# Zoe187419/ATE_replication_causalML

Measured on AMD Instinct MI355X. Metric: rows/sec for DML-ATE cross-fit, N=1e7 p=500, 1/2/4/8 MI355X; ATE/SE parity, higher is better.
Workload: dtype bf16; 1 GPU; model=DML-PLR 5-fold cross-fit, CV-LASSO nuisances (100 lambdas, inner 4-fold CV), global_batch=10000000, seq_len=500, N=10000000, p=500, folds=5, parallelism=dp1, dgp=tutorial, n_kept=10000000, layout=blocked64+bytes8

## Files before the change

ate_replication_causalml_amd/_native.py:

```python
from __future__ import annotations

import ctypes
import os
from pathlib import Path

_LIBDIR = Path(__file__).resolve().parent / "_lib"
_hip = None
_cpu = None


class NativeMissing(RuntimeError):
    pass


class NativeError(RuntimeError):

    def __init__(self, name: str, status: int, detail: str):
        self.entry, self.status = name, status
        super().__init__(f"{name} failed with status {status}: {detail}")


HIP_ERRORS = {
    1: "hipErrorInvalidValue", 2: "hipErrorOutOfMemory", 3: "hipErrorNotInitialized",
    4: "hipErrorDeinitialized", 9: "hipErrorInvalidConfiguration",
    13: "hipErrorInvalidSymbol", 17: "hipErrorInvalidDevicePointer",
    21: "hipErrorInvalidMemcpyDirection", 35: "hipErrorInsufficientDriver",
    52: "hipErrorMissingConfiguration", 53: "hipErrorPriorLaunchFailure",
    98: "hipErrorInvalidDeviceFunction", 100: "hipErrorNoDevice", 101: "hipErrorInvalidDevice",
    200: "hipErrorInvalidImage", 201: "hipErrorInvalidContext", 209: "hipErrorNoBinaryForGpu",
    218: "hipErrorInvalidKernelFile", 400: "hipErrorInvalidHandle", 500: "hipErrorNotFound",
    600: "hipErrorNotReady", 700: "hipErrorIllegalAddress", 701: "hipErrorLaunchOutOfResources",
    702: "hipErrorLaunchTimeOut", 710: "hipErrorAssert", 719: "hipErrorLaunchFailure",
    720: "hipErrorCooperativeLaunchTooLarge", 801: "hipErrorNotSupported",
    900: "hipErrorStreamCaptureUnsupported", 901: "hipErrorStreamCaptureInvalidated",
    907: "hipErrorCapturedEvent", 999: "hipErrorUnknown",
}


def describe_status(rc: int) -> str:
    if rc < 0:
        return "rejected by the entry point's own argument check (no kernel launched)"
    return f"{HIP_ERRORS.get(rc, 'hipError?')} ({rc})"


c_void_p = ctypes.c_void_p
c_int = ctypes.c_int
c_int64 = ctypes.c_int64
c_uint64 = ctypes.c_uint64
c_double = ctypes.c_double

_SIGS = {
    "ate_gram_bf16": "pliipipipipppp",
    "ate_gram_bf16_pair": "pllipippipippippiip",
    "ate_last_error": "pi",
    "ate_last_stale_error": "pi",
    "ate_clear_errors": "",
    "ate_debug_bad_launch": "ip",
    "ate_check_kernel_resources": "pi",
    "ate_gram_f32": "plippipipippppp",
    "ate_gram_f64": "plippipipippppp",
    "ate_gram_tile_sizes": "pppp",
    "ate_chol_solve": "pipiipdpppppp",
    "ate_chol_solve_k": "pipipidppppp",
    "ate_spd_solve_batched": "ppiippp",
    "ate_predict": "ipllppiidipp",
    "ate_irls_update": "ipllppiiiiippppipp",
    "ate_irls_check": "piidippp",
    "ate_naive": "ippplpppp",
    "ate_clip_propensity": "pplpp",
    "ate_aipw": "ppppppldpppp",
    "ate_dml_moments": "ppplppp",
    "ate_dml_finalize": "pipp",
    "ate_boot_multinomial": "ppluiipp",
    "ate_boot_poisson": "ppluiilipp",
    "ate_enet_prepare": "piipipiipipipppppppp",
    "ate_enet_prepare_fused": "piipipiipipi" + "ppppppp" + "plp",
    "ate_enet_prepare_fused_clear": "piipipiipipi" + "ppppppp" + "pl" + "pl" + "p",
    "ate_enet_path": "pipiippppidddipppppippp",
    "ate_enet_coef": "ppiiiipppppppp",
    "ate_enet_cvloss_gauss": "pippiipppiiipp",
    "ate_cv_select": "pppiipippppip",
    "ate_enet_pick": "ppiiipppip",
    "ate_enet_cv_tail": "pippiipppi" + "pppppp" + "iiii" + "pppppppppppp",
    "ate_dml_resid_moments": "ipllpipipiiiiiippp",
    "ate_dml_resid_moments_final": "ipllpipipiiiiii" + "ppppp",
    "ate_dml_resid_exact": "pllpipipiiiiiiippp",
    "ate_dml_resid_terms": "ipllpipipiiiiii" + "ppp",
    "ate_cluster_chunk": "",
    "ate_cluster_work": "l",
    "ate_cluster_moments": "pplpplipppp",
    "ate_irm_score_moments": "ipllpipiipiiiiidippp",
    "ate_irm_score_moments_multi": "ipllpipiipipiiiiiidippp",
    "ate_irm_score_multi_smax": "",
    "ate_irm_scores": "ipllpipiipiiiiidipp",
    "ate_irm_sens_moments": "ipllpipiipiiiiidippp",
    "ate_irm_target_moments": "ipllpipiipiiiiidippp",
    "ate_irm_score_link": "ii" + "ipllpipiipiiiiidippp",
    "ate_iivm_moments": "ipllpipiipiiiiiiidippp",
    "ate_apo_moments": "ipllpipiipiiiiidippp",
    "ate_pliv_lds_max": "",
    "ate_pliv_moments": "ipllpipiippii" + "pppp",
    "ate_pliv_terms": "ipllpipiippii" + "pppp",
    "ate_group_boot": "pppliiuippp",
    "ate_group_boot_scratch": "iii",
    "ate_cate_moments": "ppplpiiippp",
    "ate_cate_moments_scratch": "iii",
    "ate_cate_boot": "ppplppiiiuippp",
    "ate_cate_boot_scratch": "iiii",
    "ate_policy_pair_hist": "ppppppliiipp",
    "ate_policy_pair_hist_scratch": "i",
    "ate_policy_search": "ppiilppp",
    "ate_lognet_path": "iplpiipipipdddippippppppppp",
    "ate_lognet_cvloss": "iplpiippipppipp",
    "ate_lognet_path_groups": "iplpiipipipppdpdiippppppppp",
    "ate_lognet_cvloss_set": "iplpiipipipppipp",
    "ate_dgp_fill": "iplllllp" + "uiipppp",
    "ate_sel_block_rows": "",
    "ate_sel_gen_count": "upilllpp",
    "ate_sel_gen_flags": "upillpp",
    "ate_sel_gen_mark": "upiplllpiplp",
    "ate_forest_fit": "pppppi" + "pppppppp" + "ip",
    "ate_forest_predict": "ppiiipppppippip",
    "ate_forest_pack": "pippppppp",
    "ate_forest_scratch_bytes": "ii",
    "ate_forest_exact_scratch_bytes": "iiii",
    "ate_forest_fit_exact": "piiipppippppippppppppp",
    "ate_forest_predict16": "ppiiipppppppippip",
    "ate_bin_matrix": "plipppp",
    "ate_panel_xtv": "iplpipplipp",
    "ate_select_compact": "plppddpppp" + "p",
    "ate_gbdt_run": "ppp",
    "ate_lv_boot": "ppp",
    "ate_lv_classify": "pipiippp",
    "ate_lv_decide": "ppipipipippppp" + "iipip",
    "ate_lv_partition": "ppipippppipp",
    "ate_lv_scatter": "pppppippp",
    "ate_lv_children": "pippppp",
    "ate_lv_transpose": "piipip",
    "ate_gbdt_bin_panel": "pilpipppilpppl" + "p",
    "ate_gbdt_slab_entries": "liii",
    "ate_gbdt_slab2_entries": "li",
    "ate_gbdt_pair_root": "pppplllp",
    "ate_gbdt_apply": "plliipppp" + "p",
    "ate_panel_xv": "iplpipiplpp",
    "ate_col_moments": "pllipppp",
    "ate_standardize": "pllippp",
    "ate_interactions": "pllipl" + "p",
    "ate_scan_parts": "l",
    "ate_gbdt_limits": "p",
    "ate_excl_scan_i32": "plpppp",
    "ate_excl_scan_i64": "plpppp",
}
_RESTYPE = {"ate_forest_scratch_bytes": ctypes.c_int64,
            "ate_forest_exact_scratch_bytes": ctypes.c_int64, "ate_gbdt_slab_entries": ctypes.c_int64,
            "ate_gbdt_slab2_entries": ctypes.c_int64,
            "ate_scan_parts": ctypes.c_int64, "ate_group_boot_scratch": ctypes.c_int64,
            "ate_cate_moments_scratch": ctypes.c_int64,
            "ate_cate_boot_scratch": ctypes.c_int64,
            "ate_policy_pair_hist_scratch": ctypes.c_int64,
            "ate_cluster_work": ctypes.c_int64}
_CT = {"p": c_void_p, "i": c_int, "l": c_int64, "u": c_uint64, "d": c_double}


def _load(path: Path, sigs: dict):
    lib = ctypes.CDLL(str(path), mode=ctypes.RTLD_GLOBAL)
    for name, sig in sigs.items():
        if hasattr(lib, name):
            f = getattr(lib, name)
            f.restype = _RESTYPE.get(name, c_int)
            f.argtypes = [_CT[ch] for ch in sig]
    return lib


def hip_available() -> bool:
    return (_LIBDIR / "libatehip.so").exists()


def hip_library_path() -> Path:
    debug = os.environ.get("ATE_DEBUG", "0") not in ("", "0")
    return Path(os.environ["ATE_HIP_LIB"]) if os.environ.get("ATE_HIP_LIB") else \
        _LIBDIR / ("libatehip_debug.so" if debug else "libatehip.so")


def hip():
    global _hip
    if _hip is None:
        import torch
        debug = os.environ.get("ATE_DEBUG", "0") not in ("", "0")
        p = hip_library_path()
        if not p.exists():
            raise NativeMissing(
                f"{p} not found: build it with `python -m ate_replication_causalml_amd._build` "
                "(hipcc --offload-arch=gfx950). GPU ops have no fallback.")
        _hip = _load(p, _SIGS)
        if debug:
            _check_kernel_resources(_hip)
    return _hip


_resource_report = None


def _check_kernel_resources(lib):
    global _resource_report
    buf = ctypes.create_string_buffer(1 << 14)
    bad = lib.ate_check_kernel_resources(buf, len(buf))
    _resource_report = buf.value.decode(errors="replace")
    if bad > 0:
        raise NativeError("ate_check_kernel_resources", bad,
                          "kernels that cannot launch as registered:\n" + "\n".join(
                              l for l in _resource_report.splitlines() if "FAIL" in l))


def kernel_resource_report() -> str | None:
    return _resource_report


def _native_message(lib, fn: str) -> tuple[int, str]:
    buf = ctypes.create_string_buffer(512)
    code = getattr(lib, fn)(buf, len(buf))
    return code, buf.value.decode(errors="replace")


def cpu():
    global _cpu
    if _cpu is None:
        p = _LIBDIR / "libatecpu.so"
        if not p.exists():
            from ._build import build_cpu
            build_cpu()
        _cpu = _load(p, {})
    return _cpu


def check(rc: int, name: str = "native call"):
    if rc != 0:
        raise RuntimeError(f"{name} failed with code {rc}")


def call(name: str, *args):
    lib = hip()
    rc = getattr(lib, name)(*args)
    if rc != 0:
        raise NativeError(name, rc, status_detail(lib, rc))
    return rc


def status_detail(lib, rc: int) -> str:
    detail = describe_status(rc)
    if rc > 0 and hasattr(lib, "ate_last_error"):
        code, msg = _native_message(lib, "ate_last_error")
        if code == rc and msg:
            detail = msg
        scode, smsg = _native_message(lib, "ate_last_stale_error")
        if scode and smsg:
            detail += f" [stale, cleared before the launch: {smsg}]"
        lib.ate_clear_errors()
    return detail


def loaded_libraries():
    out = []
    try:
        with open(f"/proc/{os.getpid()}/maps") as f:
            for line in f:
                if str(_LIBDIR) in line:
                    out.append(line.split()[-1])
    except OSError:
        pass
    return sorted(set(out))
```

ate_replication_causalml_amd/data/device_dgp.py:

```python
from __future__ import annotations

import os

import numpy as np
import torch

from .. import _native
from ..ops.panel import DevicePanel, empty_panel, dtype_code
from . import dgp as host_dgp

N_TUTORIAL_COLS = 21
DGPS = ("tutorial", "tutorial-rct", "rct")


def fold_slices(n_total: int, folds: int, rank: int = 0, world: int = 1, align: int = 0):
    out = []
    for k in range(folds):
        f0, f1 = k * n_total // folds, (k + 1) * n_total // folds
        m = f1 - f0
        if align:
            nb = -(-m // align)
            a = min(f1, f0 + (rank * nb // world) * align)
            b = min(f1, f0 + ((rank + 1) * nb // world) * align)
        else:
            a = f0 + rank * m // world
            b = f0 + (rank + 1) * m // world
        out.append((a, b - a))
    return out


BYTE_COL0 = 384
BYTE_PANEL = os.environ.get("ATE_PANEL_BYTES", "1") == "1"


def _binary_names(p: int) -> set:
    out = {"one", "W", "Y", "W_hi", "W_lo", "Y_hi", "Y_lo"}
    out |= {f"x{j}" for j in range(15, min(21, p))}
    out |= {f"x{j}" for j in range(21, p) if (j - 21) % 4 == 3}
    return out


def byte_column_order(names: list, p: int, P: int):
    if P != 512:
        return None
    binary = _binary_names(p)
    cont = [nm for nm in names if nm not in binary]
    if len(cont) > BYTE_COL0:
        return None
    return cont + [nm for nm in names if nm in binary]


def _arm_split_ids(base: DevicePanel):
    w = base.col("W").double()
    counts, gparts, rows = [], [], []
    off = 0
    for (r0, _), cnt in zip(base.seg_bounds, base.seg_nreal):
        r0, cnt = int(r0), int(cnt)
        wk = w[r0:r0 + cnt]
        rk = base.row_index[r0:r0 + cnt]
        gk = rk if base.gen_ids is None else base.gen_ids[off:off + cnt]
        off += cnt
        for a in (0, 1):
            ix = torch.nonzero(wk == a).reshape(-1)
            counts.append(int(ix.numel()))
            gparts.append(gk[ix])
            rows.append(rk[ix])
    if sum(counts) != base.n:
        raise ValueError("arm_split needs a binary W column")
    return counts, torch.cat(gparts).contiguous(), rows, base.selection


def synthetic_panel(n_total: int, p: int = 500, folds: int = 5, seed: int = 1991,
                    dtype: str = "bf16", device="cpu", rank: int = 0, world: int = 1,
                    blocked: bool = False, align: int = 0, dgp: str = "rct", comm=None,
                    selection=None, compat: str = "reference",
                    arm_split: bool = False) -> DevicePanel:
    if p < N_TUTORIAL_COLS:
        raise ValueError("p must be >= 21 (tutorial columns)")
    if dgp not in DGPS:
        raise ValueError(f"dgp must be one of {DGPS}, got {dgp!r}")
    if comm is not None:
        rank, world = comm.rank, comm.world_size
    p_extra = p - N_TUTORIAL_COLS
    params = host_dgp.PANEL if dgp == "rct" else host_dgp.TUTORIAL
    if arm_split and align:
        raise ValueError("arm_split panels are not block-aligned: align must be 0")
    slices = fold_slices(n_total, folds, rank, world, align)
    split = None
    if arm_split:
        split = _arm_split_ids(synthetic_panel(
            n_total, p=p, folds=folds, seed=seed, dtype=dtype, device=device, rank=rank,
            world=world, blocked=blocked, dgp=dgp, comm=comm, selection=selection, compat=compat))
        slices = [(0, c) for c in split[0]]
    hi_lo = dtype == "bf16"
    names = ["one"] + [f"x{j}" for j in range(p)] + ["W", "Y"]
    if hi_lo:
        names += ["W_hi", "W_lo", "Y_hi", "Y_lo"]
    cpad = 128 if dtype == "bf16" else 64
    P = (len(names) + cpad - 1) // cpad * cpad
    pan = empty_panel([c for _, c in slices], P, dtype=dtype, device=device, blocked=blocked)
    order = byte_column_order(names, p, P) if (
        hi_lo and blocked and pan.data.is_cuda and BYTE_PANEL) else None
    pan.cols = {nm: i for i, nm in enumerate(names if order is None else order)}
    pan.xcols = [pan.cols[f"x{j}"] for j in range(p)]
    pcol = None
    if order is not None:
        pcol = torch.as_tensor([pan.cols[nm] for nm in names], dtype=torch.int16,
                               device=pan.data.device)
        pan.bytes8 = torch.zeros((pan.ld // 64, P - BYTE_COL0, 64), dtype=torch.uint8,
                                 device=pan.data.device)
    rid = torch.full((pan.ld,), -1, dtype=torch.int64, device=device)
    for (g0, cnt), (r0, _) in zip(slices, pan.seg_bounds):
        rid[r0:r0 + cnt] = torch.arange(g0, g0 + cnt, device=device)
    pan.row_index = rid
    pan.identity = len(slices) == 1 and slices[0][0] == 0
    gids = None
    sel = None
    if split is not None:
        _, gids, rows, sel = split
        for k, (r0, _) in enumerate(pan.seg_bounds):
            rid[r0:r0 + int(split[0][k])] = rows[k]
    elif dgp == "tutorial":
        from .panel_selection import kept_gids, plan_selection
        pcomm = None if getattr(comm, "emulated", False) else comm
        sel = selection if selection is not None else plan_selection(
            n_total, seed, params, comm=pcomm, device=pan.data.device, compat=compat)
        if sel.n_keep != n_total or sel.seed != seed:
            raise ValueError("selection plan does not match (n_total, seed)")
        if sel.compat != compat or sel.params != params:
            raise ValueError(f"selection plan made for compat={sel.compat!r} / other DGP "
                             f"parameters, not compat={compat!r}")
        gids = kept_gids(sel, slices, device=pan.data.device)
    offs = np.concatenate([[0], np.cumsum([c for _, c in slices])])
    if pan.data.is_cuda:
        s = torch.cuda.current_stream().cuda_stream
        pblk = np.ascontiguousarray(params.device_block())
        for k, ((g0, cnt), (r0, _)) in enumerate(zip(slices, pan.seg_bounds)):
            gp = 0 if gids is None or cnt == 0 else gids[int(offs[k]):].data_ptr()
            _native.call("ate_dgp_fill", dtype_code(pan.data), pan.data.data_ptr(),
                         *pan.strides(), int(r0), cnt, g0, gp, seed, p_extra, int(hi_lo),
                         pblk.ctypes.data, None if pcol is None else pcol.data_ptr(),
                         None if pcol is None else pan.bytes8.data_ptr(), s)
    else:
        cm = torch.zeros((pan.P, pan.ld), dtype=pan.data.dtype) if blocked else pan.data
        for k, ((g0, cnt), (r0, _)) in enumerate(zip(slices, pan.seg_bounds)):
            idx = None if gids is None else gids[int(offs[k]):int(offs[k]) + cnt].numpy()
            cts, binc, extra, W, Y, _ = host_dgp.raw_columns(cnt, seed, p_extra, row_offset=g0,
                                                              params=params, idx=idx)
            cols = [np.ones(cnt), *cts.T, *binc.T, *extra.T, W, Y]
            if hi_lo:
                cols += [W, np.zeros(cnt), Y, np.zeros(cnt)]
            block = torch.from_numpy(np.stack(cols)).to(pan.data.dtype)
            cm[:block.shape[0], r0:r0 + cnt] = block
        if blocked:
            pan.data.copy_(cm.reshape(pan.P, -1, 64).permute(1, 0, 2))
    pan.n = sum(c for _, c in slices)
    pan.exact_block = int(align)
    pan.dgp = dgp
    pan.selection = sel
    pan.n_generated = sel.n_gen if sel is not None else n_total
    pan.gen_ids = gids
    return pan
```

ate_replication_causalml_amd/ops/gram.py:

```python
from __future__ import annotations

import contextlib
import os

import numpy as np
import torch

from .. import _native
from ..utils.graphs import pin
from .panel import DevicePanel

BF16_TILE, BF16_K = 128, 64
BF16_TILE_BIG = 256
SMALL_TILE, SMALL_K = 64, 16
TARGET_WG = 2048

GRAM_KERNEL = os.environ.get("ATE_GRAM_KERNEL", "pair")
PAIR_SLOTS = 272
BYTE_COLS = os.environ.get("ATE_GRAM_BYTES", "1") == "1"
SCHEDULES = {"lockstep": 0, "stagger": 1}
GRAM_SCHED = os.environ.get("ATE_GRAM_SCHED", "stagger")
GRAM_PRIO = int(os.environ.get("ATE_GRAM_PRIO", "-1"))
PLAN_CACHE_MAX = int(os.environ.get("ATE_GRAM_PLAN_CACHE", 8))

_plan_cache: dict = {}
_slot = 0


@contextlib.contextmanager
def plan_slot(i: int):
    global _slot
    prev, _slot = _slot, int(i)
    try:
        yield
    finally:
        _slot = prev


def _stream():
    return torch.cuda.current_stream().cuda_stream


class GramPlan:
    def __init__(self, panel: DevicePanel, weighted: bool, exact: bool = False):
        bf16 = panel.dtype == torch.bfloat16
        if bf16 and weighted:
            raise ValueError("weighted Gram needs an fp32/fp64 panel")
        P = panel.P
        self.pair = bf16 and P % (2 * BF16_TILE_BIG) == 0 and GRAM_KERNEL == "pair"
        if bf16:
            T = BF16_TILE_BIG if P % BF16_TILE_BIG == 0 else BF16_TILE
        else:
            T = SMALL_TILE
        K = BF16_K if bf16 else SMALL_K
        if P % T:
            raise ValueError(f"panel P={P} must be a multiple of {T}")
        nt = P // T
        if self.pair:
            tiles, blocks = _pair_tiles(nt)
        else:
            tiles = [(a, b) for a in range(nt) for b in range(a, nt)]
        ntiles = len(tiles)
        rows_total = int((panel.seg_bounds[:, 1] - panel.seg_bounds[:, 0]).sum())
        target = 3072 if T == BF16_TILE_BIG else TARGET_WG
        whole_rounds = False
        if self.pair:
            env = os.environ.get("ATE_GRAM_PAIR_WG")
            whole_rounds = env is None
            rounds = int(os.environ.get("ATE_GRAM_ROUNDS", "5"))
            target = int(env) if env is not None else rounds * _cu_count(panel.device)
        target = int(os.environ.get("ATE_GRAM_WG", target))
        nchunk_target = max(1, target // ntiles)
        chunks = []
        seg_chunk0 = [0]
        if exact:
            B = int(panel.exact_block)
            if B <= 0 or B % K:
                raise ValueError("exact Gram needs a block-aligned panel (synthetic_panel("
                                 f"align=B) with B a multiple of {K})")
            for s_, (r0, r1) in enumerate(panel.seg_bounds):
                r = int(r0)
                while r < r1:
                    e = min(int(r1), r + B)
                    chunks.append((r, e, s_, 0))
                    r = e
                seg_chunk0.append(len(chunks))
        elif self.pair:
            chunks, seg_chunk0 = pair_chunks(panel.seg_bounds, K, ntiles, target,
                                             _cu_count(panel.device) if whole_rounds else 0)
        else:
            ch_rows = max(K, (rows_total // nchunk_target) // K * K)
            for s, (r0, r1) in enumerate(panel.seg_bounds):
                r = int(r0)
                while r < r1:
                    e = min(int(r1), r + ch_rows)
                    chunks.append((r, e, s, 0))
                    r = e
                seg_chunk0.append(len(chunks))
        dev = panel.device
        self.T, self.K, self.ntiles, self.nchunks = T, K, ntiles, len(chunks)
        self.tiles = torch.tensor(tiles, dtype=torch.int32, device=dev)
        if self.pair:
            self.blocks = torch.tensor(blocks, dtype=torch.int32, device=dev)
        ch = np.zeros(len(chunks), dtype=[("r0", "<i8"), ("r1", "<i8"), ("seg", "<i4"),
                                          ("pad", "<i4")])
        for i, c in enumerate(chunks):
            ch[i] = c
        self.chunks = torch.from_numpy(ch.view(np.uint8).copy()).to(dev)
        self.seg_chunk0 = torch.tensor(seg_chunk0, dtype=torch.int32, device=dev)
        slab_dtype = torch.float32 if panel.dtype != torch.float64 else torch.float64
        per_tile = PAIR_SLOTS * 256 if self.pair else T * T
        self.slab = torch.empty(self.nchunks * ntiles * per_tile, dtype=slab_dtype, device=dev)
        self.G = torch.empty((panel.nseg, P, P), dtype=torch.float64, device=dev)
        self.Gx = torch.empty((2, panel.nseg, P, P), dtype=torch.int64, device=dev) \
            if exact else None


def pair_chunks(seg_bounds, K: int, ntiles: int, target: int, ncu: int = 0):
    nseg = max(1, len(seg_bounds))
    k = max(1, max(1, target // ntiles) // nseg)
    if ncu > 0:
        per = ntiles * nseg
        kr = k
        while kr > 1 and (per * kr) % ncu:
            kr -= 1
        if (per * kr) % ncu == 0 and 2 * kr >= k:
            k = kr
    chunks, seg_chunk0 = [], [0]
    for s, (r0, r1) in enumerate(seg_bounds):
        r0, r1 = int(r0), int(r1)
        steps = (r1 - r0) // K
        ks = max(1, min(k, steps))
        for j in range(ks):
            a = r0 + (steps * j // ks) * K
            e = r0 + (steps * (j + 1) // ks) * K if j + 1 < ks else r1
            chunks.append((a, e, s, 0))
        seg_chunk0.append(len(chunks))
    return chunks, seg_chunk0


def _cu_count(dev) -> int:
    try:
        return int(torch.cuda.get_device_properties(dev).multi_processor_count)
    except Exception:
        return 256


def _pair_tiles(nt: int):
    tiles = []
    for a in range(0, nt - 1, 2):
        tiles.append((a, a + 1, 0, 0))
        tiles.append((a, a + 1, 1, 0))
    if nt % 2:
        tiles.append((nt - 1, nt - 1, 2, 0))
    paired = {(a, a + 1) for a in range(0, nt - 1, 2)}
    tiles += [(a, b, 0, 0) for a in range(nt) for b in range(a + 1, nt) if (a, b) not in paired]
    blocks = []
    for (a, b, typ, _) in tiles:
        tb = [(-1, -1)] * PAIR_SLOTS
        if typ == 0:
            for w in range(8):
                wr, wc = w >> 2, w & 3
                for m in range(8):
                    for n in range(4):
                        tb[w * 32 + m * 4 + n] = (a * 16 + wr * 8 + m, b * 16 + wc * 4 + n)
        else:
            rs, ts = 32, 36
            for w in range(4):
                region, half = w >> 1, w & 1
                if typ == 2 and region == 1:
                    continue
                base = (a if region == 0 else b) * 16
                for m in range(8):
                    for n in range(4):
                        tb[w * rs + m * 4 + n] = (base + m, base + 8 + half * 4 + n)
            for w in range(4):
                region, half = w >> 1, w & 1
                if typ == 2 and region == 1:
                    continue
                base = (a if region == 0 else b) * 16 + half * 8
                idx = 0
                for m in range(8):
                    for n in range(m, 8):
                        tb[4 * rs + w * ts + idx] = (base + m, base + n)
                        idx += 1
        blocks.append(tb)
    return tiles, blocks


def plan_for(panel: DevicePanel, weighted=False, exact=False) -> GramPlan:
    key = (panel.data.data_ptr(), tuple(panel.data.shape), panel.data.dtype, weighted,
           tuple(map(tuple, panel.seg_bounds)), _slot, exact)
    pl = _plan_cache.pop(key, None)
    if pl is None:
        while len(_plan_cache) >= PLAN_CACHE_MAX:
            _plan_cache.pop(next(iter(_plan_cache)))
        pl = GramPlan(panel, weighted, exact)
    _plan_cache[key] = pl
    return pin(pl)


def clear_plans():
    _plan_cache.clear()


_STAGES = {"all": 3, "tiles": 1, "reduce": 2}


def _sched_for(cs: int) -> int:
    return SCHEDULES[GRAM_SCHED] if cs < (1 << 28) else SCHEDULES["lockstep"]


EXACT_LIMB_BOUND = 2.0 ** 38


def check_exact_range(panel: DevicePanel, n_total: int | None = None, w=None, comm=None):
    X = panel.data
    if X.is_cuda and torch.cuda.is_current_stream_capturing():
        return
    dims = (0, 2) if panel.blocked else 1
    amax = torch.maximum(X.amax(dim=dims), -X.amin(dim=dims)).double()
    m = torch.stack([amax.max(), w.abs().max().double() if w is not None
                     else torch.ones((), dtype=torch.float64, device=amax.device)])
    if comm is not None and comm.world_size > 1:
        comm.all_reduce_max_(m)
    xm, wm = (float(v) for v in m.cpu())
    bound = xm ** 2 * float(n_total or panel.n)
    if w is not None:
        bound *= wm
    if not bound < EXACT_LIMB_BOUND:
        raise ValueError(f"exact Gram: entries up to {bound:.3g} exceed the int64 limb range "
                         f"(2^38 = {EXACT_LIMB_BOUND:.3g}); rescale the columns or use the "
                         "non-exact mode")


def gram(panel: DevicePanel, w: torch.Tensor | None = None, done: torch.Tensor | None = None,
         out: torch.Tensor | None = None, stage: str = "all", exact: bool = False,
         n_total: int | None = None, checked: bool = False) -> torch.Tensor:
    X = panel.data
    if exact and stage != "reduce" and not checked:
        check_exact_range(panel, n_total, w)
    if not X.is_cuda:
        if exact:
            return _gram_cpu_exact(panel, w)
        return _gram_cpu(panel, w, out) if stage != "reduce" else out
    pl = plan_for(panel, weighted=w is not None, exact=exact)
    G = pl.G if out is None else out
    Gx = pl.Gx.data_ptr() if exact else None
    s = _stream()
    if X.dtype == torch.bfloat16 and pl.pair:
        cs, bs = panel.strides()
        x8 = getattr(panel, "bytes8", None)
        _native.call("ate_gram_bf16_pair", X.data_ptr(), cs, bs, panel.P, pl.tiles.data_ptr(),
                     pl.ntiles, pl.blocks.data_ptr(), pl.chunks.data_ptr(), pl.nchunks,
                     pl.seg_chunk0.data_ptr(), panel.nseg, pl.slab.data_ptr(), G.data_ptr(),
                     _STAGES[stage], Gx, None if x8 is None or not BYTE_COLS else x8.data_ptr(),
                     _sched_for(cs), GRAM_PRIO, s)
        return pl.Gx if exact else G
    if stage == "reduce":
        return pl.Gx if exact else G
    if X.dtype == torch.bfloat16:
        _native.call("ate_gram_bf16", X.data_ptr(), panel.cm_ld, panel.P, pl.T, pl.tiles.data_ptr(),
                     pl.ntiles, pl.chunks.data_ptr(), pl.nchunks, pl.seg_chunk0.data_ptr(),
                     panel.nseg, pl.slab.data_ptr(), G.data_ptr(), Gx, s)
    else:
        name = "ate_gram_f64" if X.dtype == torch.float64 else "ate_gram_f32"
        if w is not None:
            assert w.dtype == X.dtype and w.numel() == panel.ld
        _native.call(name, X.data_ptr(), panel.cm_ld, panel.P, 0 if w is None else w.data_ptr(),
                     pl.tiles.data_ptr(), pl.ntiles, pl.chunks.data_ptr(), pl.nchunks,
                     pl.seg_chunk0.data_ptr(), panel.nseg, pl.slab.data_ptr(), G.data_ptr(),
                     0 if done is None else done.data_ptr(), Gx, s)
    return pl.Gx if exact else G


def _gram_cpu(panel, w, out):
    X = panel.colmajor().double()
    Gs = []
    for (r0, r1) in panel.seg_bounds:
        Xs = X[:, r0:r1]
        A = Xs if w is None else Xs * w[r0:r1].double()
        Gs.append(A @ Xs.T)
    G = torch.stack(Gs)
    if out is not None:
        out.copy_(G)
        return out
    return G


def _gram_cpu_exact(panel, w):
    from .exact import to_limbs
    B = int(panel.exact_block)
    if B <= 0:
        raise ValueError("exact Gram needs a block-aligned panel (synthetic_panel(align=B))")
    X = panel.colmajor().double()
    out = torch.zeros((2, panel.nseg, panel.P, panel.P), dtype=torch.int64)
    for s_, (r0, r1) in enumerate(panel.seg_bounds):
        for r in range(int(r0), int(r1), B):
            e = min(int(r1), r + B)
            Xs = X[:, r:e]
            A = Xs if w is None else Xs * w[r:e].double()
            out[:, s_] += to_limbs(A @ Xs.T)
    return out


def gram_reference(panel: DevicePanel, w=None) -> torch.Tensor:
    X = panel.colmajor().double().cpu()
    wv = None if w is None else w.double().cpu()
    out = []
    for (r0, r1) in panel.seg_bounds:
        Xs = X[:, r0:r1]
        A = Xs if wv is None else Xs * wv[r0:r1]
        out.append(A @ Xs.T)
    return torch.stack(out)
```

ate_replication_causalml_amd/ops/panel.py:

```python
from __future__ import annotations

from dataclasses import dataclass, field

import numpy as np
import torch

ROW_ALIGN = 64


def _dtype(name):
    return {"bf16": torch.bfloat16, "f32": torch.float32, "f64": torch.float64}[name]


def dtype_code(t: torch.Tensor) -> int:
    return {torch.float32: 1, torch.float64: 2, torch.bfloat16: 3}[t.dtype]


@dataclass
class DevicePanel:
    data: torch.Tensor
    n: int
    cols: dict
    seg_bounds: np.ndarray
    seg_nreal: np.ndarray
    row_index: torch.Tensor
    xcols: list = field(default_factory=list)
    identity: bool = False
    blocked: bool = False
    exact_block: int = 0
    bytes8: torch.Tensor | None = None

    @property
    def P(self):
        return self.data.shape[1] if self.blocked else self.data.shape[0]

    @property
    def ld(self):
        return self.data.shape[0] * ROW_ALIGN if self.blocked else self.data.shape[1]

    @property
    def cm_ld(self):
        if self.blocked:
            raise NotImplementedError("this kernel reads column-major panels only; build the "
                                      "panel with blocked=False")
        return self.data.shape[1]

    def strides(self):
        return (ROW_ALIGN, ROW_ALIGN * self.P) if self.blocked else (self.ld, ROW_ALIGN)

    @property
    def device(self):
        return self.data.device

    @property
    def dtype(self):
        return self.data.dtype

    @property
    def nseg(self):
        return len(self.seg_bounds)

    def col(self, name) -> torch.Tensor:
        c = self.cols[name]
        return self.data[:, c, :].reshape(-1) if self.blocked else self.data[c]

    def valid(self) -> torch.Tensor:
        return self.col("one")

    def colmajor(self) -> torch.Tensor:
        if not self.blocked:
            return self.data
        return self.data.permute(1, 0, 2).reshape(self.P, self.ld)

    def gather_rows(self, v: torch.Tensor) -> torch.Tensor:
        out = torch.zeros(self.ld, dtype=v.dtype, device=self.device)
        if self.identity:
            out[:self.n] = v.to(self.device)
            return out
        m = self.row_index >= 0
        out[m] = v.to(self.device)[self.row_index[m]]
        return out

    def scatter_rows(self, v: torch.Tensor) -> torch.Tensor:
        if self.identity:
            return v[:self.n].clone()
        m = self.row_index >= 0
        out = torch.empty((self.n,) + tuple(v.shape[1:]), dtype=v.dtype, device=v.device)
        out[self.row_index[m]] = v[m]
        return out


def _round_up(x, m):
    return (x + m - 1) // m * m


def build_panel(X, W=None, Y=None, folds=None, dtype="f64", device="cpu", extra_cols=(),
                col_align=None, split_hi_lo=None, nseg=None, targets=None) -> DevicePanel:
    Xt = None
    if isinstance(X, torch.Tensor):
        Xt = X.to(device=device, dtype=torch.float64)
        if Xt.ndim == 1:
            Xt = Xt[:, None]
        X = np.empty(tuple(Xt.shape), dtype=np.float64)
    X = np.asarray(X, dtype=np.float64)
    if X.ndim == 1:
        X = X[:, None]
    n, p = X.shape
    tdt = _dtype(dtype)
    if split_hi_lo is None:
        split_hi_lo = dtype == "bf16"
    if col_align is None:
        col_align = 128 if dtype == "bf16" else 64
    names = ["one"] + [f"x{j}" for j in range(p)]
    vecs = {}
    if W is not None:
        names.append("W")
        vecs["W"] = np.asarray(W, float)
    if Y is not None:
        names.append("Y")
        vecs["Y"] = np.asarray(Y, float)
    if split_hi_lo:
        for k in list(vecs):
            names += [f"{k}_hi", f"{k}_lo"]
    for k, v in (targets or {}).items():
        if k in names or k in extra_cols or len(np.shape(v)) != 1 or len(v) != n:
            raise ValueError(f"target column {k!r}: a new name and {n} values are needed")
        names.append(k)
        vecs[k] = np.asarray(v, float)
        if split_hi_lo:
            names += [f"{k}_hi", f"{k}_lo"]
    names += list(extra_cols)
    P = _round_up(len(names), col_align)
    if folds is None:
        folds = np.zeros(n, dtype=np.int64)
    folds = np.asarray(folds, dtype=np.int64)
    K = max(int(folds.max()) + 1 if n else 1, int(nseg or 0))
    order = np.argsort(folds, kind="stable")
    counts = np.bincount(folds, minlength=K)
    padded = np.array([_round_up(max(c, 1), ROW_ALIGN) for c in counts])
    starts = np.concatenate([[0], np.cumsum(padded)[:-1]])
    ld = int(padded.sum())
    row_index = np.full(ld, -1, dtype=np.int64)
    pos = 0
    for k in range(K):
        rows = order[pos:pos + counts[k]]
        row_index[starts[k]:starts[k] + counts[k]] = rows
        pos += counts[k]
    m = row_index >= 0
    ri = row_index[m]
    host = np.zeros((P if Xt is None else P - p, ld), dtype=np.float64)
    hrow = (lambda r: r) if Xt is None else (lambda r: r if r == 0 else r - p)
    host[0, m] = 1.0
    if Xt is None:
        host[1:1 + p, m] = X[ri].T
    c = 1 + p
    cols = {n_: i for i, n_ in enumerate(names)}
    for k, v in vecs.items():
        host[hrow(cols[k]), m] = v[ri]
    if split_hi_lo:
        for k, v in vecs.items():
            hi = torch.from_numpy(v[ri]).to(torch.bfloat16).double().numpy()
            lo = v[ri] - hi
            host[hrow(cols[f"{k}_hi"]), m] = hi
            host[hrow(cols[f"{k}_lo"]), m] = lo
    if Xt is None:
        data = torch.from_numpy(host).to(tdt).to(device)
    else:
        data = torch.empty((P, ld), dtype=tdt, device=device)
        rest = torch.from_numpy(host).to(tdt).to(device)
        data[:1] = rest[:1]
        data[1 + p:] = rest[1:]
        blk = torch.zeros((p, ld), dtype=torch.float64, device=device)
        blk[:, torch.from_numpy(np.flatnonzero(m)).to(device)] = \
            Xt[torch.from_numpy(ri).to(device)].T
        data[1:1 + p] = blk.to(tdt)
    seg_bounds = np.stack([starts, starts + padded], axis=1)
    return DevicePanel(data=data, n=n, cols=cols, seg_bounds=seg_bounds,
                       seg_nreal=counts.astype(np.int64),
                       row_index=torch.from_numpy(row_index).to(device),
                       xcols=[cols[f"x{j}"] for j in range(p)], identity=K == 1)


def empty_panel(n_per_seg, P, dtype="bf16", device="cpu", blocked=False):
    counts = np.asarray(n_per_seg, dtype=np.int64)
    padded = np.array([_round_up(max(int(c), 1), ROW_ALIGN) for c in counts])
    starts = np.concatenate([[0], np.cumsum(padded)[:-1]])
    ld = int(padded.sum())
    shape = (ld // ROW_ALIGN, P, ROW_ALIGN) if blocked else (P, ld)
    data = torch.zeros(shape, dtype=_dtype(dtype), device=device)
    row_index = torch.full((ld,), -1, dtype=torch.int64, device=device)
    base = 0
    for s, c in zip(starts, counts):
        row_index[s:s + c] = torch.arange(base, base + c, device=device)
        base += int(c)
    return DevicePanel(data=data, n=int(counts.sum()), cols={"one": 0},
                       seg_bounds=np.stack([starts, starts + padded], axis=1),
                       seg_nreal=counts, row_index=row_index, identity=len(counts) == 1,
                       blocked=blocked)
```

ate_replication_causalml_amd/utils/graphs.py:

```python
from __future__ import annotations

import contextlib
import gc

import torch

_pins: list | None = None


@contextlib.contextmanager
def _no_gc():
    was = gc.isenabled()
    gc.disable()
    try:
        yield
    finally:
        if was:
            gc.enable()


def pin(obj):
    if _pins is not None:
        _pins.append(obj)
    return obj


class GraphedStep:
    def __init__(self, fn, warmup: int = 1):
        global _pins
        self.fn = fn
        for _ in range(warmup):
            fn()
        torch.cuda.synchronize()
        self.graph = torch.cuda.CUDAGraph()
        prev, _pins = _pins, []
        try:
            gc.collect()
            with _no_gc(), torch.cuda.graph(self.graph):
                self.out = fn()
            self.pins = _pins
        finally:
            _pins = prev
        torch.cuda.synchronize()

    def __call__(self):
        self.graph.replay()
        return self.out


def maybe_graphed(fn, enable: bool, warmup: int = 1):
    if not enable or not torch.cuda.is_available():
        return fn, False
    try:
        return GraphedStep(fn, warmup), True
    except Exception as e:
        print(f"[graphs] capture failed, running eagerly: {e}", flush=True)
        torch.cuda.synchronize()
        return fn, False


class Collective:

    def __init__(self, fn, capturable: bool = False):
        self.fn = fn
        self.capturable = capturable

    def __call__(self, state):
        return self.fn(state)


def _fuse(phases, fuse_collectives=False):
    out, run = [], []

    def flush():
        if run:
            fns = tuple(run)

            def composed(st, fns=fns):
                for f in fns:
                    st = f(st)
                return st
            out.append(composed)
            run.clear()

    for ph in phases:
        if isinstance(ph, Collective) and not (fuse_collectives and ph.capturable):
            flush()
            out.append(ph)
        else:
            run.append(ph)
    flush()
    return out


class SegmentedStep:

    def __init__(self, phases, graph: bool, warmup: int = 1, capture_collectives: bool = True,
                 agree=None):
        self.raw = list(phases)
        self.fallback_reason = None
        has_cc = any(isinstance(p, Collective) and p.capturable for p in self.raw)
        self.phases = _fuse(self.raw)
        self.graphs = [None] * len(self.phases)
        self.pins = []
        self.collectives_captured = False
        for _ in range(warmup):
            self._eager()
        if not graph:
            return
        if capture_collectives and has_cc:
            ok, err = True, None
            try:
                self._capture(_fuse(self.raw, fuse_collectives=True), replay=False)
            except Exception as e:
                ok, err = False, e
            if agree is not None:
                ok = bool(agree(ok))
                if err is None and not ok:
                    err = RuntimeError("another rank could not capture its collectives")
            if ok:
                self()
                torch.cuda.synchronize()
                self.collectives_captured = True
                return
            self.fallback_reason = repr(err)
            print(f"[graphs] capturing the collectives failed, they run eagerly between "
                  f"graph segments: {err}", flush=True)
            torch.cuda.synchronize()
            self.phases = _fuse(self.raw)
            self.graphs = [None] * len(self.phases)
            self.pins = []
        self._capture(_fuse(self.raw))

    def _capture(self, phases, replay: bool = True):
        global _pins
        torch.cuda.synchronize()
        graphs = [None] * len(phases)
        pins = []
        state = None
        for i, ph in enumerate(phases):
            if isinstance(ph, Collective):
                state = ph(state)
                continue
            g = torch.cuda.CUDAGraph()
            prev, _pins = _pins, []
            try:
                gc.collect()
                with _no_gc(), torch.cuda.graph(g):
                    out = ph(state)
                pins += _pins
            finally:
                _pins = prev
            graphs[i] = (g, out)
            torch.cuda.synchronize()
            if replay:
                g.replay()
            state = out
        torch.cuda.synchronize()
        self.phases, self.graphs, self.pins = phases, graphs, pins

    @property
    def graphed(self) -> bool:
        return any(g is not None for g in self.graphs)

    @property
    def graph_count(self) -> int:
        return sum(g is not None for g in self.graphs)

    def _eager(self):
        state = None
        for ph in self.phases:
            state = ph(state)
        return state

    def __call__(self):
        state = None
        for ph, g in zip(self.phases, self.graphs):
            if g is None:
                state = ph(state)
            else:
                g[0].replay()
                state = g[1]
        return state


def _data(x):
    return x if isinstance(x, torch.Tensor) else x.data


def layout_key(*inputs):
    key = []
    for x in inputs:
        if x is None:
            key.append(None)
            continue
        t = _data(x)
        k = (tuple(t.shape), t.dtype, str(t.device))
        if not isinstance(x, torch.Tensor):
            k += (x.n, tuple(sorted(x.cols.items())), tuple(map(tuple, x.seg_bounds)),
                  tuple(int(c) for c in x.seg_nreal), bool(getattr(x, "identity", False)),
                  getattr(x, "bytes8", None) is not None)
        key.append(k)
    return tuple(key)


class _Captured:

    def __init__(self, body, inputs, static_args, warmup):
        self.inputs = inputs = list(inputs)
        self.step = GraphedStep(lambda: body(*inputs, *static_args), warmup)

    def load(self, inputs):
        for s, x in zip(self.inputs, inputs):
            if x is not s and x is not None:
                _data(s).copy_(_data(x))
                if getattr(x, "bytes8", None) is not None:
                    s.bytes8.copy_(x.bytes8)

    def __call__(self, inputs):
        self.load(inputs)
        return self.step()


class _Seen:

    def __init__(self, inputs):
        self.inputs = None if inputs is None else list(inputs)


def _nbytes(inputs):
    tot = 0
    for x in inputs:
        if x is None:
            continue
        t = _data(x)
        tot += t.numel() * t.element_size()
    return tot


def _env_bytes(name, default):
    import os
    v = os.environ.get(name)
    return int(float(v)) if v else default


class GraphCache:

    def __init__(self, maxsize: int = 32, max_bytes: int | None = None,
                 retain_bytes: int | None = None):
        self.maxsize = maxsize
        self.max_bytes = max_bytes if max_bytes is not None else \
            _env_bytes("ATE_GRAPH_CACHE_BYTES", 24 << 30)
        self.retain_bytes = retain_bytes if retain_bytes is not None else \
            _env_bytes("ATE_GRAPH_RETAIN_BYTES", 1 << 30)
        self.entries: dict = {}
        self.sizes: dict = {}
        self.eager: set = set()

    @property
    def held_bytes(self):
        return sum(self.sizes.values())

    def _evict(self, need=0):
        while self.entries and (len(self.entries) >= self.maxsize or
                                self.held_bytes + need > self.max_bytes):
            k = next(iter(self.entries))
            self.entries.pop(k)
            self.sizes.pop(k, None)

    def run(self, name, body, inputs, *static_args):
        key = (name, static_args, layout_key(*inputs))
        if key in self.eager:
            return body(*inputs, *static_args), False
        g = self.entries.pop(key, None)
        self.sizes.pop(key, None)
        nb = _nbytes(inputs)
        if g is None:
            keep = nb <= self.retain_bytes and nb <= self.max_bytes
            self._evict(nb if keep else 0)
            self.entries[key] = _Seen(inputs if keep else None)
            self.sizes[key] = nb if keep else 0
            return body(*inputs, *static_args), False
        if isinstance(g, _Seen):
            if nb > self.max_bytes:
                self.entries[key] = g
                self.sizes[key] = 0
                return body(*inputs, *static_args), False
            self._evict(nb)
            static = g.inputs if g.inputs is not None else list(inputs)
            try:
                torch.cuda.synchronize()
                for s, x in zip(static, inputs):
                    if x is not s and x is not None:
                        _data(s).copy_(_data(x))
                        if getattr(x, "bytes8", None) is not None:
                            s.bytes8.copy_(x.bytes8)
                g = _Captured(body, static, static_args, warmup=1)
            except Exception as e:
                print(f"[graphs] {name}: capture failed, running eagerly: {e}", flush=True)
                torch.cuda.synchronize()
                self.eager.add(key)
                return body(*inputs, *static_args), False
        self.entries[key] = g
        self.sizes[key] = nb
        return g(inputs), True

    def drop(self, name, inputs, *static_args):
        key = (name, static_args, layout_key(*inputs))
        self.entries.pop(key, None)
        self.sizes.pop(key, None)
        self.eager.discard(key)

    def clear(self):
        self.entries.clear()
        self.sizes.clear()
        self.eager.clear()


estimator_graphs = GraphCache()


def clear_graph_caches():
    estimator_graphs.clear()
    try:
        from ..ops.gram import clear_plans
        clear_plans()
    except Exception:
        pass
    if torch.cuda.is_available():
        torch.cuda.empty_cache()
```

csrc/dgp.hip:

```cpp
#include "common.hpp"

using namespace ate;

namespace {

struct DgpP {
  float intercept, b_hist[5], b_latent, tau_logit, p_treat, thr[5], hist_latent, yob_latent,
      factor_load, factor_rest;
  int uniform_b;
  double p_treat_d, thr_d[5], hist_latent_d, yob_latent_d;
};

DgpP load_params(const double* a) {
  DgpP P;
  P.p_treat_d = a[8];
  for (int k = 0; k < 5; ++k) P.thr_d[k] = a[9 + k];
  P.hist_latent_d = a[14];
  P.yob_latent_d = a[15];
  P.intercept = a[0];
  for (int k = 0; k < 5; ++k) P.b_hist[k] = a[1 + k];
  P.b_latent = a[6];
  P.tau_logit = a[7];
  P.p_treat = a[8];
  for (int k = 0; k < 5; ++k) P.thr[k] = a[9 + k];
  P.hist_latent = a[14];
  P.yob_latent = a[15];
  P.factor_load = a[16];
  P.factor_rest = a[17];
  P.uniform_b = 1;
  for (int k = 1; k < 5; ++k) P.uniform_b &= (P.b_hist[k] == P.b_hist[0]);
  return P;
}

__device__ __forceinline__ float dgp_normal(uint64_t seed, uint32_t stream, uint64_t idx) {
  u32x4 w = rand4(seed, P_DGP, stream, idx);
  float u1 = ((float)(w.x >> 8) + 1.0f) * (1.0f / 16777217.0f);
  float u2 = (float)(w.y >> 8) * (1.0f / 16777216.0f);
  return sqrtf(-2.0f * logf(u1)) * cosf(6.283185307179586f * u2);
}
__device__ __forceinline__ float dgp_uniform(uint64_t seed, uint32_t stream, uint64_t idx) {
  u32x4 w = rand4(seed, P_DGP, stream, idx);
  return (float)(w.x >> 8) * (1.0f / 16777216.0f);
}
__device__ __forceinline__ double dgp_normal_d(uint64_t seed, uint32_t stream, uint64_t idx) {
#pragma clang fp contract(off)
  u32x4 w = rand4(seed, P_DGP, stream, idx);
  const double u1 = ((double)(w.x >> 8) + 1.0) * (1.0 / 16777217.0);
  const double u2 = (double)(w.y >> 8) * (1.0 / 16777216.0);
  return sqrt(-2.0 * log(u1)) * cos(6.283185307179586 * u2);
}
__device__ __forceinline__ double dgp_uniform_d(uint64_t seed, uint32_t stream, uint64_t idx) {
  u32x4 w = rand4(seed, P_DGP, stream, idx);
  return (double)(w.x >> 8) * (1.0 / 16777216.0);
}

struct Core {
  double yob, city, latent;
  float w;
  int hist;
};

__device__ __forceinline__ Core core_draws(uint64_t seed, uint64_t g, const DgpP& P) {
#pragma clang fp contract(off)
  Core c;
  c.yob = dgp_normal_d(seed, 0, g);
  c.city = dgp_normal_d(seed, 1, g);
  c.latent = dgp_normal_d(seed, 41, g) + P.yob_latent_d * c.yob;
  c.hist = 0;
#pragma unroll
  for (int k = 0; k < 5; ++k)
    c.hist |= (dgp_normal_d(seed, 50 + k, g) + P.hist_latent_d * c.latent > P.thr_d[k])
                  ? (1 << k) : 0;
  c.w = dgp_uniform_d(seed, 61, g) < P.p_treat_d ? 1.f : 0.f;
  return c;
}

__device__ __forceinline__ int sel_flag(const Core& c, int last) {
  const int h = c.hist;
  if (c.w == 1.f) {
    const bool d = (h & 0xF) != 0 || ((h >> last) & 1) || c.city > 2.0 || c.yob > 2.0;
    return d ? 1 : 0;
  }
  const bool d = (h & 0x1F) != 0x1F || c.city < -2.0 || c.yob < -2.0;
  return d ? 2 : 0;
}

__device__ __forceinline__ int64_t pidx(int c, int64_t i, int64_t cs, int64_t bs) {
  return (int64_t)c * cs + (i >> 6) * bs + (i & 63);
}
template <typename T>
__device__ __forceinline__ void put(T* X, int64_t cs, int64_t bs, int c, int64_t i, float v) {
  X[pidx(c, i, cs, bs)] = (T)v;
}
template <>
__device__ __forceinline__ void put<bf16_t>(bf16_t* X, int64_t cs, int64_t bs, int c, int64_t i,
                                            float v) {
  X[pidx(c, i, cs, bs)] = f32_to_bf16_rne(v);
}
template <typename T>
__device__ __forceinline__ void put_d(T* X, int64_t cs, int64_t bs, int c, int64_t i, double v) {
  if constexpr (sizeof(T) == 8) X[pidx(c, i, cs, bs)] = (T)v;
  else put(X, cs, bs, c, i, (float)v);
}

constexpr int X8_COL0 = 384;
__device__ __forceinline__ int x8_pos(int64_t i) {
  const int r = (int)(i & 63);
  return ((r >> 3) & 3) * 16 + (r >> 5) * 8 + (r & 7);
}

template <typename T>
__global__ void dgp_fill_kernel(T* __restrict__ X, int64_t cs, int64_t bs, int64_t row0, int64_t count,
                                int64_t gid0, const int64_t* __restrict__ gids, uint64_t seed,
                                int p_extra, int hi_lo, DgpP P, const int16_t* __restrict__ pcol,
                                uint8_t* __restrict__ X8) {
  const float FL = P.factor_load, FS = P.factor_rest;
  for (int64_t r = blockIdx.x * (int64_t)blockDim.x + threadIdx.x; r < count;
       r += (int64_t)gridDim.x * blockDim.x) {
    const uint64_t g = gids != nullptr ? (uint64_t)gids[r] : (uint64_t)(gid0 + r);
    const int64_t i = row0 + r;
    const Core cr = core_draws(seed, g, P);
    const float f = dgp_normal(seed, 40, g);
    int c = 0;
    auto phys = [&](int cl) { return pcol != nullptr ? (int)pcol[cl] : cl; };
    auto emit = [&](float v) {
      const int pc = phys(c++);
      put(X, cs, bs, pc, i, v);
      if (X8 != nullptr && pc >= X8_COL0) {
        ATE_DASSERT(v == 0.f || v == 1.f);
        X8[(i >> 6) * (128 * 64) + (pc - X8_COL0) * 64 + x8_pos(i)] = v != 0.f ? 0x3F : 0;
      }
    };
    emit(1.0f);
    ATE_DASSERT(phys(1) < X8_COL0 || X8 == nullptr);
    put_d(X, cs, bs, phys(c++), i, cr.yob);
    put_d(X, cs, bs, phys(c++), i, cr.city);
    for (int j = 2; j < 15; ++j) {
      float z = dgp_normal(seed, j, g);
      emit(j < 3 ? z : FL * f + FS * z);
    }
    const float sex = dgp_uniform(seed, 60, g) < 0.5f ? 1.f : 0.f;
    emit(sex);
    float hsum = 0.f, hb = 0.f;
#pragma unroll
    for (int k = 0; k < 5; ++k) {
      const float h = ((cr.hist >> k) & 1) ? 1.f : 0.f;
      hsum += h;
      hb += P.b_hist[k] * h;
      emit(h);
    }
    for (int j = 0; j < p_extra; ++j) {
      float z = dgp_normal(seed, 100 + j, g);
      float v = (j % 4 == 3) ? (z > 0.f ? 1.f : 0.f) : FL * f + FS * z;
      emit(v);
    }
    const float w = cr.w;
    const float hterm = P.uniform_b ? P.b_hist[0] * hsum : hb;
    const float eta = P.intercept + hterm + P.b_latent * (float)cr.latent + P.tau_logit * w;
    const float y = dgp_uniform(seed, 62, g) < 1.0f / (1.0f + expf(-eta)) ? 1.f : 0.f;
    emit(w);
    emit(y);
    if (hi_lo) {
      emit(w);
      emit(0.f);
      emit(y);
      emit(0.f);
    }
  }
}

constexpr int NT = 256;
constexpr int SEL_BR = 16384;

__global__ __launch_bounds__(NT) void sel_gen_count_kernel(uint64_t seed, DgpP P, int last,
                                                           int64_t b0, int64_t n_lim,
                                                           int64_t* __restrict__ cnt) {
  __shared__ int ws[2][NT / 64];
  const int64_t b = b0 + blockIdx.x;
  const int64_t g0 = b * SEL_BR;
  int ct = 0, cc = 0;
  for (int k = threadIdx.x; k < SEL_BR; k += NT) {
    const int64_t g = g0 + k;
    if (g >= n_lim) break;
    const int f = sel_flag(core_draws(seed, (uint64_t)g, P), last);
    ct += f == 1;
    cc += f == 2;
  }
  ct = wave_sum(ct);
  cc = wave_sum(cc);
  const int lane = threadIdx.x & 63, wid = threadIdx.x >> 6;
  if (lane == 0) { ws[0][wid] = ct; ws[1][wid] = cc; }
  __syncthreads();
  if (threadIdx.x == 0) {
    int64_t t = 0, c = 0;
    for (int w = 0; w < NT / 64; ++w) { t += ws[0][w]; c += ws[1][w]; }
    cnt[2 * blockIdx.x] = t;
    cnt[2 * blockIdx.x + 1] = c;
  }
}

__global__ __launch_bounds__(NT) void sel_gen_flags_kernel(uint64_t seed, DgpP P, int last,
                                                           int64_t g0, int64_t count,
                                                           uint8_t* __restrict__ flags) {
  for (int64_t r = blockIdx.x * (int64_t)NT + threadIdx.x; r < count; r += (int64_t)gridDim.x * NT)
    flags[r] = (uint8_t)sel_flag(core_draws(seed, (uint64_t)(g0 + r), P), last);
}

__device__ int block_scan(int x, int* ws) {
  const int lane = threadIdx.x & 63, wid = threadIdx.x >> 6;
  int incl = x;
#pragma unroll
  for (int o = 1; o < 64; o <<= 1) {
    const int t = __shfl_up(incl, o, 64);
    if (lane >= o) incl += t;
  }
  if (lane == 63) ws[wid] = incl;
  __syncthreads();
  int off = 0, tot = 0;
  for (int w = 0; w < NT / 64; ++w) {
    if (w < wid) off += ws[w];
    tot += ws[w];
  }
  __syncthreads();
  if (threadIdx.x == 0) ws[NT / 64] = tot;
  __syncthreads();
  return off + incl - x;
}

__global__ __launch_bounds__(NT) void sel_gen_mark_kernel(uint64_t seed, DgpP P, int last,
                                                          const int64_t* __restrict__ blk,
                                                          int64_t thr_t, int64_t thr_c,
                                                          const int64_t* __restrict__ sl, int ns,
                                                          int64_t* __restrict__ out, int64_t cap) {
  __shared__ int ws[3][NT / 64 + 1];
  const int64_t* B = blk + 6 * (int64_t)blockIdx.x;
  const int64_t g0 = B[0], g1 = B[1];
  int64_t ct = B[2], cc = B[3], kp = B[4];
  ATE_DASSERT(g1 - g0 <= SEL_BR && g0 <= g1);
  for (int64_t base = g0; base < g1; base += NT) {
    const int64_t g = base + threadIdx.x;
    const int f = g < g1 ? sel_flag(core_draws(seed, (uint64_t)g, P), last) : 0;
    const int et = block_scan(f == 1, ws[0]);
    const int ec = block_scan(f == 2, ws[1]);
    const bool drop = (f == 1 && ct + et < thr_t) || (f == 2 && cc + ec < thr_c);
    const int k = g < g1 && !drop;
    const int ek = block_scan(k, ws[2]);
    if (k) {
      const int64_t q = kp + ek;
      for (int s = 0; s < ns; ++s) {
        if (q >= sl[3 * s] && q < sl[3 * s + 1]) {
          const int64_t o = sl[3 * s + 2] + (q - sl[3 * s]);
          ATE_DASSERT(o >= 0 && o < cap);
          out[o] = g;
          break;
        }
      }
    }
    ct += ws[0][NT / 64];
    cc += ws[1][NT / 64];
    kp += ws[2][NT / 64];
  }
}

}

ATE_API int ate_dgp_fill(int dtype, void* X, int64_t cs, int64_t bs, int64_t row0, int64_t count,
                         int64_t gid0, const void* gids, uint64_t seed, int p_extra, int hi_lo,
                         const void* params, const void* pcol, void* X8, void* stream) {
  hipStream_t s = (hipStream_t)stream;
  const DgpP P = load_params((const double*)params);
  const int64_t* gl = (const int64_t*)gids;
  const int16_t* pc = (const int16_t*)pcol;
  dim3 grid(grid_for(count, 256, 8192)), block(256);
  if (X8 != nullptr && dtype != 3) return -1;
  if (dtype == 1)
    ATE_LAUNCH(dgp_fill_kernel<float>, grid, block, 0, s, (float*)X, cs, bs, row0, count, gid0,
                       gl, seed, p_extra, hi_lo, P, pc, (uint8_t*)nullptr);
  else if (dtype == 2)
    ATE_LAUNCH(dgp_fill_kernel<double>, grid, block, 0, s, (double*)X, cs, bs, row0, count,
                       gid0, gl, seed, p_extra, hi_lo, P, pc, (uint8_t*)nullptr);
  else if (dtype == 3)
    ATE_LAUNCH(dgp_fill_kernel<bf16_t>, grid, block, 0, s, (bf16_t*)X, cs, bs, row0, count,
                       gid0, gl, seed, p_extra, hi_lo, P, pc, (uint8_t*)X8);
  else
    return -1;
  ATE_CHECK_LAUNCH();
  return 0;
}

ATE_API int ate_sel_block_rows() { return SEL_BR; }

ATE_API int ate_sel_gen_count(uint64_t seed, const void* params, int last, int64_t b0, int64_t nblk,
                              int64_t n_lim, void* cnt, void* stream) {
  if (nblk <= 0) return 0;
  const DgpP P = load_params((const double*)params);
  ATE_LAUNCH(sel_gen_count_kernel, dim3((unsigned)nblk), dim3(NT), 0, (hipStream_t)stream,
                     seed, P, last, b0, n_lim, (int64_t*)cnt);
  ATE_CHECK_LAUNCH();
  return 0;
}

ATE_API int ate_sel_gen_flags(uint64_t seed, const void* params, int last, int64_t g0, int64_t count,
                              void* flags, void* stream) {
  if (count <= 0) return 0;
  const DgpP P = load_params((const double*)params);
  ATE_LAUNCH(sel_gen_flags_kernel, dim3(grid_for(count, NT, 4096)), dim3(NT), 0,
                     (hipStream_t)stream, seed, P, last, g0, count, (uint8_t*)flags);
  ATE_CHECK_LAUNCH();
  return 0;
}

ATE_API int ate_sel_gen_mark(uint64_t seed, const void* params, int last, const void* blk, int64_t nl,
                             int64_t thr_t, int64_t thr_c, const void* sl, int ns, void* out,
                             int64_t cap, void* stream) {
  if (nl <= 0) return 0;
  const DgpP P = load_params((const double*)params);
  ATE_LAUNCH(sel_gen_mark_kernel, dim3((unsigned)nl), dim3(NT), 0, (hipStream_t)stream,
                     seed, P, last, (const int64_t*)blk, thr_t, thr_c, (const int64_t*)sl, ns,
                     (int64_t*)out, cap);
  ATE_CHECK_LAUNCH();
  return 0;
}
```

csrc/gram.hip:

```cpp
#include "common.hpp"

using namespace ate;

struct Chunk { int64_t row0, row1; int seg, pad; };

__device__ __forceinline__ int xcd_remap(int bid, int nwg) {
  int xcd = bid & 7, q = nwg >> 3, r = nwg & 7;
  int base = (xcd < r) ? xcd * (q + 1) : r * (q + 1) + (xcd - r) * q;
  return base + (bid >> 3);
}

constexpr int BT = 128;
constexpr int BK = 64;

__global__ __launch_bounds__(256) void gram_bf16_kernel(
    const bf16_t* __restrict__ X, int64_t ld, const int2* __restrict__ tiles, int ntiles,
    const Chunk* __restrict__ chunks, int nchunks, float* __restrict__ slab) {
  __shared__ __attribute__((aligned(16))) bf16_t lds[2][2][BT * BK];
  const int L = xcd_remap(blockIdx.x, gridDim.x);
  const int c = L / ntiles, t = L % ntiles;
  const Chunk ch = chunks[c];
  const int2 tl = tiles[t];
  const bool diag = tl.x == tl.y;
  const int a0 = tl.x * BT, b0 = tl.y * BT;
  const int tid = threadIdx.x, lane = tid & 63, wid = tid >> 6;
  const int wr = wid >> 1, wc = wid & 1;

  f32x4 acc[4][4];
#pragma unroll
  for (int i = 0; i < 4; ++i)
#pragma unroll
    for (int j = 0; j < 4; ++j) acc[i][j] = f32x4{0.f, 0.f, 0.f, 0.f};

  uint4 ra[4], rb[4];
  auto gload = [&](int64_t i0) {
#pragma unroll
    for (int r = 0; r < 4; ++r) {
      int idx = r * 256 + tid, col = idx >> 3, cc = idx & 7;
      ra[r] = *reinterpret_cast<const uint4*>(X + (int64_t)(a0 + col) * ld + i0 + cc * 8);
      if (!diag) rb[r] = *reinterpret_cast<const uint4*>(X + (int64_t)(b0 + col) * ld + i0 + cc * 8);
    }
  };
  auto lstore = [&](int buf) {
#pragma unroll
    for (int r = 0; r < 4; ++r) {
      int idx = r * 256 + tid, col = idx >> 3, cc = idx & 7;
      int off = col * BK + ((cc ^ (col & 7)) << 3);
      *reinterpret_cast<uint4*>(&lds[buf][0][off]) = ra[r];
      if (!diag) *reinterpret_cast<uint4*>(&lds[buf][1][off]) = rb[r];
    }
  };

  const int64_t nsteps = (ch.row1 - ch.row0) / BK;
  if (nsteps > 0) {
    gload(ch.row0);
    lstore(0);
  }
  __syncthreads();
  for (int64_t s = 0; s < nsteps; ++s) {
    const int buf = s & 1;
    if (s + 1 < nsteps) gload(ch.row0 + (s + 1) * BK);
    const bf16_t* As = lds[buf][0];
    const bf16_t* Bs = diag ? lds[buf][0] : lds[buf][1];
#pragma unroll
    for (int kk = 0; kk < 2; ++kk) {
      const int cc = kk * 4 + (lane >> 4);
      bf16x8 af[4], bfr[4];
#pragma unroll
      for (int m = 0; m < 4; ++m) {
        int col = wr * 64 + m * 16 + (lane & 15);
        af[m] = *reinterpret_cast<const bf16x8*>(&As[col * BK + ((cc ^ (col & 7)) << 3)]);
      }
#pragma unroll
      for (int n = 0; n < 4; ++n) {
        int col = wc * 64 + n * 16 + (lane & 15);
        bfr[n] = *reinterpret_cast<const bf16x8*>(&Bs[col * BK + ((cc ^ (col & 7)) << 3)]);
      }
#pragma unroll
      for (int m = 0; m < 4; ++m)
#pragma unroll
        for (int n = 0; n < 4; ++n)
          acc[m][n] = __builtin_amdgcn_mfma_f32_16x16x32_bf16(af[m], bfr[n], acc[m][n], 0, 0, 0);
    }
    if (s + 1 < nsteps) lstore(buf ^ 1);
    __syncthreads();
  }
  float* out = slab + ((int64_t)c * ntiles + t) * (BT * BT);
#pragma unroll
  for (int m = 0; m < 4; ++m)
#pragma unroll
    for (int n = 0; n < 4; ++n)
#pragma unroll
      for (int r = 0; r < 4; ++r) {
        int row = wr * 64 + m * 16 + (lane >> 4) * 4 + r;
        int col = wc * 64 + n * 16 + (lane & 15);
        out[row * BT + col] = acc[m][n][r];
      }
}

constexpr int GT = 256;
constexpr int GK = 64;

typedef const __attribute__((address_space(1))) char* gptr_t;
__device__ __forceinline__ void glds16(gptr_t src, bf16_t* lds_base) {
  __builtin_amdgcn_global_load_lds(src, (__attribute__((address_space(3))) void*)(lds_base), 16, 0, 0);
}
__device__ __forceinline__ void glds16(const void* src, bf16_t* lds_base) {
  __builtin_amdgcn_global_load_lds(src, (__attribute__((address_space(3))) void*)(lds_base), 16, 0, 0);
}

__global__ __launch_bounds__(512) void gram_bf16_256_kernel(
    const bf16_t* __restrict__ X, int64_t ld, const int2* __restrict__ tiles, int ntiles,
    const Chunk* __restrict__ chunks, int nchunks, float* __restrict__ slab) {
  __shared__ __attribute__((aligned(16))) bf16_t lds[2][2][GT * GK];
  const int L = xcd_remap(blockIdx.x, gridDim.x);
  const int c = L / ntiles, t = L % ntiles;
  const Chunk ch = chunks[c];
  const int2 tl = tiles[t];
  const bool diag = tl.x == tl.y;
  const int a0 = tl.x * GT, b0 = tl.y * GT;
  const int tid = threadIdx.x, lane = tid & 63, wid = tid >> 6;
  const int wr = wid >> 2, wc = wid & 3;

  f32x4 acc[8][4];
#pragma unroll
  for (int i = 0; i < 8; ++i)
#pragma unroll
    for (int j = 0; j < 4; ++j) acc[i][j] = f32x4{0.f, 0.f, 0.f, 0.f};

  auto stage = [&](int st, int64_t i0) {
#pragma unroll
    for (int r = 0; r < 4; ++r) {
      const int q = wid * 4 + r;
      const int col = q * 8 + (lane >> 3);
      const int cc = (lane & 7) ^ (col & 7);
      glds16(X + (int64_t)(a0 + col) * ld + i0 + cc * 8, &lds[st][0][q * 8 * GK]);
      if (!diag) glds16(X + (int64_t)(b0 + col) * ld + i0 + cc * 8, &lds[st][1][q * 8 * GK]);
    }
  };

  const int64_t nsteps = (ch.row1 - ch.row0) / GK;
  if (nsteps > 0) stage(0, ch.row0);
  __builtin_amdgcn_s_waitcnt(0x0F70);
  __syncthreads();
  for (int64_t s = 0; s < nsteps; ++s) {
    const int cur = s & 1;
    if (s + 1 < nsteps) stage(cur ^ 1, ch.row0 + (s + 1) * GK);
    const bf16_t* As = lds[cur][0];
    const bf16_t* Bs = diag ? lds[cur][0] : lds[cur][1];
#pragma unroll
    for (int kk = 0; kk < 2; ++kk) {
      const int cc = kk * 4 + (lane >> 4);
      bf16x8 af[8], bfr[4];
#pragma unroll
      for (int m = 0; m < 8; ++m) {
        const int col = wr * 128 + m * 16 + (lane & 15);
        af[m] = *reinterpret_cast<const bf16x8*>(&As[col * GK + ((cc ^ (col & 7)) << 3)]);
      }
#pragma unroll
      for (int n = 0; n < 4; ++n) {
        const int col = wc * 64 + n * 16 + (lane & 15);
        bfr[n] = *reinterpret_cast<const bf16x8*>(&Bs[col * GK + ((cc ^ (col & 7)) << 3)]);
      }
#pragma unroll
      for (int m = 0; m < 8; ++m)
#pragma unroll
        for (int n = 0; n < 4; ++n)
          acc[m][n] = __builtin_amdgcn_mfma_f32_16x16x32_bf16(af[m], bfr[n], acc[m][n], 0, 0, 0);
    }
    __builtin_amdgcn_s_waitcnt(0x0F70);
    __syncthreads();
  }
  float* out = slab + ((int64_t)c * ntiles + t) * (GT * GT);
#pragma unroll
  for (int m = 0; m < 8; ++m)
#pragma unroll
    for (int n = 0; n < 4; ++n)
#pragma unroll
      for (int r = 0; r < 4; ++r) {
        const int row = wr * 128 + m * 16 + (lane >> 4) * 4 + r;
        const int col = wc * 64 + n * 16 + (lane & 15);
        out[row * GT + col] = acc[m][n][r];
      }
}

constexpr int PAIR_SLOTS = 272;
constexpr int PAIR_LDS = 2 * 2 * GT * GK;
#ifndef GRAM_PRIO
#define GRAM_PRIO 2
#endif

__device__ __forceinline__ int tri_index(int m, int n) {
  return m * 8 - (m * (m - 1)) / 2 + (n - m);
}

constexpr int PAIR_RECT = 0, PAIR_RECT_D0 = 1, PAIR_TRI = 2, PAIR_RECT_D1 = 3;
template <int MODE> struct PairRole {
  static constexpr bool TRI = MODE == PAIR_TRI;
  static constexpr int NB = TRI ? 36 : 32;
};

template <int MODE>
__device__ __forceinline__ void pair_mfma(f32x4* acc, const bf16x8* af, const bf16x8* bfr) {
  if constexpr (MODE != PAIR_TRI) {
#pragma unroll
    for (int m = 0; m < 8; ++m)
#pragma unroll
      for (int n = 0; n < 4; ++n)
        acc[m * 4 + n] = __builtin_amdgcn_mfma_f32_16x16x32_bf16(af[m], bfr[n], acc[m * 4 + n],
                                                                 0, 0, 0);
  } else {
#pragma unroll
    for (int m = 0; m < 8; ++m)
#pragma unroll
      for (int n = m; n < 8; ++n)
        acc[tri_index(m, n)] = __builtin_amdgcn_mfma_f32_16x16x32_bf16(
            af[m], af[n], acc[tri_index(m, n)], 0, 0, 0);
  }
}

__device__ __forceinline__ bf16x8 bytes_to_bf16x8(uint2 d) {
  uint4 w;
  w.x = __builtin_amdgcn_perm(0u, d.x, 0x010C000Cu);
  w.y = __builtin_amdgcn_perm(0u, d.x, 0x030C020Cu);
  w.z = __builtin_amdgcn_perm(0u, d.y, 0x010C000Cu);
  w.w = __builtin_amdgcn_perm(0u, d.y, 0x030C020Cu);
  return __builtin_bit_cast(bf16x8, w);
}
constexpr int PAIR_BYTE0 = 384;

constexpr int SCHED_LOCKSTEP = 0, SCHED_STAGGER = 1;

template <int MODE, bool BYTES, bool BY, bool LATE, bool SADDR>
__device__ __forceinline__ void pair_wave(const bf16_t* __restrict__ X, int64_t cs, int64_t bs, int a0,
                                          int b0, bool haveB, bool idle, int abuf, int bbuf,
                                          int arow0, int bcol0, const Chunk& ch,
                                          bf16_t* lds_raw, float* __restrict__ out,
                                          const uint8_t* __restrict__ X8) {
  constexpr bool TRI = PairRole<MODE>::TRI;
  constexpr int NB = PairRole<MODE>::NB;
  const int tid = threadIdx.x, lane = tid & 63, wid = tid >> 6;
  f32x4 acc[NB];
#pragma unroll
  for (int i = 0; i < NB; ++i) acc[i] = f32x4{0.f, 0.f, 0.f, 0.f};
  bf16_t (*lds)[2][GT * GK] = reinterpret_cast<bf16_t (*)[2][GT * GK]>(lds_raw);
  const int wu = __builtin_amdgcn_readfirstlane(wid);
  const uint32_t voff_ = (uint32_t)(((lane >> 3) * cs + (((lane & 7) ^ (lane >> 3)) << 3)) * 2);
  const uint32_t voff8_ = (uint32_t)((lane >> 2) * GK + (((lane & 3) ^ ((lane >> 3) & 2)) << 4));
  auto stage = [&](int st, int64_t i0) {
    if constexpr (SADDR) {
      gptr_t Xk0 = (gptr_t) reinterpret_cast<const char*>(X + (i0 >> 6) * bs);
      uint32_t voff = voff_, voff8 = voff8_;
#if defined(__HIP_DEVICE_COMPILE__)
      asm volatile("" : "+v"(voff), "+v"(voff8));
#endif
      const int nbp = 2;
#pragma unroll
      for (int r = 0; r < 4; ++r) {
        const int q = wu * 4 + r;
        glds16(Xk0 + (int64_t)(a0 + q * 8) * cs * 2 + voff, &lds[st][0][q * 8 * GK]);
        if (!BYTES && haveB)
          glds16(Xk0 + (int64_t)(b0 + q * 8) * cs * 2 + voff, &lds[st][1][q * 8 * GK]);
      }
      if constexpr (BYTES) {
#pragma unroll
        for (int r = 0; r < nbp; ++r) {
          const int q = wu * 2 + r;
          glds16(Xk0 + (int64_t)(b0 + q * 8) * cs * 2 + voff, &lds[st][1][q * 8 * GK]);
        }
        glds16((gptr_t) reinterpret_cast<const char*>(X8) + (i0 >> 6) * (128 * GK) + wu * 1024 + voff8,
               reinterpret_cast<bf16_t*>(reinterpret_cast<uint8_t*>(&lds[st][1][128 * GK]) +
                                         wu * 1024));
      }
      return;
    }
    if constexpr (BYTES) {
      const bf16_t* Xk0 = X + (i0 >> 6) * bs;
#pragma unroll
      for (int r = 0; r < 4; ++r) {
        const int q = wid * 4 + r;
        const int col = q * 8 + (lane >> 3);
        const int cc = (lane & 7) ^ (col & 7);
        glds16(Xk0 + cc * 8 + (int64_t)(a0 + col) * cs, &lds[st][0][q * 8 * GK]);
      }
#pragma unroll
      for (int r = 0; r < 2; ++r) {
        const int q = wid * 2 + r;
        const int col = q * 8 + (lane >> 3);
        const int cc = (lane & 7) ^ (col & 7);
        glds16(Xk0 + cc * 8 + (int64_t)(b0 + col) * cs, &lds[st][1][q * 8 * GK]);
      }
      const int cb = wid * 16 + (lane >> 2);
      const int pc = (lane & 3) ^ ((cb >> 1) & 2);
      glds16(X8 + (i0 >> 6) * (128 * GK) + cb * GK + pc * 16,
             reinterpret_cast<bf16_t*>(reinterpret_cast<uint8_t*>(&lds[st][1][128 * GK]) +
                                       wid * 1024));
      return;
    }
#pragma unroll
    for (int r = 0; r < 4; ++r) {
      const int q = wid * 4 + r;
      const int col = q * 8 + (lane >> 3);
      const int cc = (lane & 7) ^ (col & 7);
      const bf16_t* Xk = X + (i0 >> 6) * bs + cc * 8;
      glds16(Xk + (int64_t)(a0 + col) * cs, &lds[st][0][q * 8 * GK]);
      if (haveB) glds16(Xk + (int64_t)(b0 + col) * cs, &lds[st][1][q * 8 * GK]);
    }
  };
  auto frag = [&](const bf16_t* P_, int col, int cc) {
    return *reinterpret_cast<const bf16x8*>(&P_[col * GK + ((cc ^ (col & 7)) << 3)]);
  };
  auto raw16 = [&](const bf16_t* P_, int col) {
    const int cb = col - 128;
    const uint8_t* b8 = reinterpret_cast<const uint8_t*>(P_ + 128 * GK);
    const int slot = (lane >> 4) ^ ((cb >> 1) & 2);
    return *reinterpret_cast<const uint4*>(b8 + cb * GK + slot * 16);
  };
  const int64_t nsteps = (ch.row1 - ch.row0) / GK;
  if (nsteps > 0) stage(0, ch.row0);
  __builtin_amdgcn_s_waitcnt(0x0F70);
  __syncthreads();
  bf16x8 ha[LATE ? 8 : 1], hb[LATE && !TRI ? 4 : 1];
  if constexpr (LATE) {
#pragma unroll
    for (int m = 0; m < 8; ++m) ha[m] = bf16x8{};
    if constexpr (!TRI) {
#pragma unroll
      for (int n = 0; n < 4; ++n) hb[n] = bf16x8{};
    }
  }
  for (int64_t s = 0; s < nsteps; ++s) {
    const int cur = s & 1;
    const bf16_t* As = lds[cur][abuf];
    const bf16_t* Bs = lds[cur][bbuf];
    if constexpr (LATE) {
      bf16x8 na[8], nb[TRI ? 1 : 4];
      uint4 raw[BY ? (TRI ? 8 : 4) : 1];
      const int c0 = lane >> 4, c1 = 4 + (lane >> 4);
      if (!idle) {
        if constexpr (BY && !TRI) {
#pragma unroll
          for (int n = 0; n < 4; ++n) raw[n] = raw16(Bs, bcol0 + n * 16 + (lane & 15));
#pragma unroll
          for (int m = 0; m < 8; ++m) na[m] = frag(As, arow0 + m * 16 + (lane & 15), c0);
          pair_mfma<MODE>(acc, ha, hb);
#pragma unroll
          for (int i = 0; i < 12; ++i) {
            __builtin_amdgcn_sched_group_barrier(0x008, 1, 0);
            __builtin_amdgcn_sched_group_barrier(0x100, 1, 0);
          }
          __builtin_amdgcn_sched_group_barrier(0x008, NB - 12, 0);
        } else if constexpr (BY) {
#pragma unroll
          for (int m = 0; m < 8; ++m) raw[m] = raw16(As, arow0 + m * 16 + (lane & 15));
#pragma unroll
          for (int m = 0; m < 8; ++m) na[m] = bytes_to_bf16x8(make_uint2(raw[m].x, raw[m].y));
          pair_mfma<MODE>(acc, ha, ha);
#pragma unroll
          for (int i = 0; i < 8; ++i) {
            __builtin_amdgcn_sched_group_barrier(0x008, 1, 0);
            __builtin_amdgcn_sched_group_barrier(0x100, 1, 0);
          }
#pragma unroll
          for (int i = 0; i < 16; ++i) {
            __builtin_amdgcn_sched_group_barrier(0x008, 1, 0);
            __builtin_amdgcn_sched_group_barrier(0x002, 2, 0);
          }
          __builtin_amdgcn_sched_group_barrier(0x008, NB - 24, 0);
        } else if constexpr (!TRI) {
#pragma unroll
          for (int m = 0; m < 8; ++m) na[m] = frag(As, arow0 + m * 16 + (lane & 15), c0);
#pragma unroll
          for (int n = 0; n < 4; ++n) nb[n] = frag(Bs, bcol0 + n * 16 + (lane & 15), c0);
          pair_mfma<MODE>(acc, ha, hb);
#pragma unroll
          for (int i = 0; i < 12; ++i) {
            __builtin_amdgcn_sched_group_barrier(0x008, 1, 0);
            __builtin_amdgcn_sched_group_barrier(0x100, 1, 0);
          }
          __builtin_amdgcn_sched_group_barrier(0x008, NB - 12, 0);
        } else {
#pragma unroll
          for (int m = 0; m < 8; ++m) na[m] = frag(As, arow0 + m * 16 + (lane & 15), c0);
          pair_mfma<MODE>(acc, ha, ha);
#pragma unroll
          for (int i = 0; i < 8; ++i) {
            __builtin_amdgcn_sched_group_barrier(0x008, 1, 0);
            __builtin_amdgcn_sched_group_barrier(0x100, 1, 0);
          }
          __builtin_amdgcn_sched_group_barrier(0x008, NB - 8, 0);
        }
      }
      if (s + 1 < nsteps) stage(cur ^ 1, ch.row0 + (s + 1) * GK);
      if (!idle) {
        if constexpr (BY && !TRI) {
#pragma unroll
          for (int m = 0; m < 8; ++m) ha[m] = frag(As, arow0 + m * 16 + (lane & 15), c1);
#pragma unroll
          for (int n = 0; n < 4; ++n) nb[n] = bytes_to_bf16x8(make_uint2(raw[n].x, raw[n].y));
#pragma unroll
          for (int n = 0; n < 4; ++n) hb[n] = bytes_to_bf16x8(make_uint2(raw[n].z, raw[n].w));
          pair_mfma<MODE>(acc, na, nb);
          __builtin_amdgcn_sched_group_barrier(0x002, 4, 0);
#pragma unroll
          for (int i = 0; i < 3; ++i) {
            __builtin_amdgcn_sched_group_barrier(0x008, 1, 0);
            __builtin_amdgcn_sched_group_barrier(0x002, 4, 0);
          }
#pragma unroll
          for (int i = 0; i < 8; ++i) {
            __builtin_amdgcn_sched_group_barrier(0x008, 1, 0);
            __builtin_amdgcn_sched_group_barrier(0x100, 1, 0);
          }
#pragma unroll
          for (int i = 0; i < 16; ++i) {
            __builtin_amdgcn_sched_group_barrier(0x008, 1, 0);
            __builtin_amdgcn_sched_group_barrier(0x002, 1, 0);
          }
          __builtin_amdgcn_sched_group_barrier(0x008, NB - 27, 0);
        } else if constexpr (BY) {
#pragma unroll
          for (int m = 0; m < 8; ++m) ha[m] = bytes_to_bf16x8(make_uint2(raw[m].z, raw[m].w));
          pair_mfma<MODE>(acc, na, na);
#pragma unroll
          for (int i = 0; i < 16; ++i) {
            __builtin_amdgcn_sched_group_barrier(0x008, 1, 0);
            __builtin_amdgcn_sched_group_barrier(0x002, 2, 0);
          }
          __builtin_amdgcn_sched_group_barrier(0x008, NB - 16, 0);
        } else if constexpr (!TRI) {
#pragma unroll
          for (int m = 0; m < 8; ++m) ha[m] = frag(As, arow0 + m * 16 + (lane & 15), c1);
#pragma unroll
          for (int n = 0; n < 4; ++n) hb[n] = frag(Bs, bcol0 + n * 16 + (lane & 15), c1);
          pair_mfma<MODE>(acc, na, nb);
#pragma unroll
          for (int i = 0; i < 12; ++i) {
            __builtin_amdgcn_sched_group_barrier(0x008, 1, 0);
            __builtin_amdgcn_sched_group_barrier(0x100, 1, 0);
          }
          __builtin_amdgcn_sched_group_barrier(0x008, NB - 12, 0);
        } else {
#pragma unroll
          for (int m = 0; m < 8; ++m) ha[m] = frag(As, arow0 + m * 16 + (lane & 15), c1);
          pair_mfma<MODE>(acc, na, na);
#pragma unroll
          for (int i = 0; i < 8; ++i) {
            __builtin_amdgcn_sched_group_barrier(0x008, 1, 0);
            __builtin_amdgcn_sched_group_barrier(0x100, 1, 0);
          }
          __builtin_amdgcn_sched_group_barrier(0x008, NB - 8, 0);
        }
      }
    } else {
      if (s + 1 < nsteps) stage(cur ^ 1, ch.row0 + (s + 1) * GK);
      if (!idle) {
        if constexpr (BY && !TRI) {
          bf16x8 af[2][8];
          uint4 braw[4];
#pragma unroll
          for (int n = 0; n < 4; ++n) braw[n] = raw16(Bs, bcol0 + n * 16 + (lane & 15));
#pragma unroll
          for (int kk = 0; kk < 2; ++kk) {
            const int cc = kk * 4 + (lane >> 4);
#pragma unroll
            for (int m = 0; m < 8; ++m) af[kk][m] = frag(As, arow0 + m * 16 + (lane & 15), cc);
          }
          bf16x8 b0v[4], b1v[4];
#pragma unroll
          for (int n = 0; n < 4; ++n) b0v[n] = bytes_to_bf16x8(make_uint2(braw[n].x, braw[n].y));
#pragma unroll
          for (int n = 0; n < 4; ++n) b1v[n] = bytes_to_bf16x8(make_uint2(braw[n].z, braw[n].w));
          pair_mfma<MODE>(acc, af[0], b0v);
          pair_mfma<MODE>(acc, af[1], b1v);
          __builtin_amdgcn_sched_group_barrier(0x100, 12, 0);
          __builtin_amdgcn_sched_group_barrier(0x002, 16, 0);
#pragma unroll
          for (int i = 0; i < 8; ++i) {
            __builtin_amdgcn_sched_group_barrier(0x008, 1, 0);
            __builtin_amdgcn_sched_group_barrier(0x100, 1, 0);
          }
#pragma unroll
          for (int i = 0; i < 16; ++i) {
            __builtin_amdgcn_sched_group_barrier(0x008, 1, 0);
            __builtin_amdgcn_sched_group_barrier(0x002, 1, 0);
          }
          __builtin_amdgcn_sched_group_barrier(0x008, 2 * NB - 24, 0);
        } else if constexpr (BY) {
          uint4 fraw[8];
#pragma unroll
          for (int m = 0; m < 8; ++m) fraw[m] = raw16(As, arow0 + m * 16 + (lane & 15));
          bf16x8 f0[8], f1[8];
#pragma unroll
          for (int m = 0; m < 8; ++m) f0[m] = bytes_to_bf16x8(make_uint2(fraw[m].x, fraw[m].y));
#pragma unroll
          for (int m = 0; m < 8; ++m) f1[m] = bytes_to_bf16x8(make_uint2(fraw[m].z, fraw[m].w));
          pair_mfma<MODE>(acc, f0, f0);
          pair_mfma<MODE>(acc, f1, f1);
          __builtin_amdgcn_sched_group_barrier(0x100, 8, 0);
          __builtin_amdgcn_sched_group_barrier(0x002, 32, 0);
#pragma unroll
          for (int i = 0; i < 16; ++i) {
            __builtin_amdgcn_sched_group_barrier(0x008, 1, 0);
            __builtin_amdgcn_sched_group_barrier(0x002, 2, 0);
          }
          __builtin_amdgcn_sched_group_barrier(0x008, 2 * NB - 16, 0);
        } else if constexpr (!TRI) {
          bf16x8 af[2][8], bfr[2][4];
#pragma unroll
          for (int kk = 0; kk < 2; ++kk) {
            const int cc = kk * 4 + (lane >> 4);
#pragma unroll
            for (int m = 0; m < 8; ++m) af[kk][m] = frag(As, arow0 + m * 16 + (lane & 15), cc);
#pragma unroll
            for (int n = 0; n < 4; ++n) bfr[kk][n] = frag(Bs, bcol0 + n * 16 + (lane & 15), cc);
          }
#pragma unroll
          for (int kk = 0; kk < 2; ++kk) pair_mfma<MODE>(acc, af[kk], bfr[kk]);
          __builtin_amdgcn_sched_group_barrier(0x100, 12, 0);
#pragma unroll
          for (int i = 0; i < 12; ++i) {
            __builtin_amdgcn_sched_group_barrier(0x008, 1, 0);
            __builtin_amdgcn_sched_group_barrier(0x100, 1, 0);
          }
          __builtin_amdgcn_sched_group_barrier(0x008, 2 * NB - 12, 0);
        } else {
          bf16x8 fr[2][8];
#pragma unroll
          for (int kk = 0; kk < 2; ++kk) {
            const int cc = kk * 4 + (lane >> 4);
#pragma unroll
            for (int m = 0; m < 8; ++m) fr[kk][m] = frag(As, arow0 + m * 16 + (lane & 15), cc);
          }
#pragma unroll
          for (int kk = 0; kk < 2; ++kk) pair_mfma<MODE>(acc, fr[kk], fr[kk]);
          __builtin_amdgcn_sched_group_barrier(0x100, 8, 0);
#pragma unroll
          for (int i = 0; i < 8; ++i) {
            __builtin_amdgcn_sched_group_barrier(0x008, 1, 0);
            __builtin_amdgcn_sched_group_barrier(0x100, 1, 0);
          }
          __builtin_amdgcn_sched_group_barrier(0x008, 2 * NB - 8, 0);
        }
      }
    }
    __builtin_amdgcn_s_waitcnt(0x0F70);
    __syncthreads();
  }
  if constexpr (LATE) {
    if (!idle) pair_mfma<MODE>(acc, ha, TRI ? ha : hb);
  }
  if (idle) return;
#pragma unroll
  for (int i = 0; i < NB; ++i)
    *reinterpret_cast<f32x4*>(out + i * 256 + lane * 4) = acc[i];
}

#ifdef GRAM_CLOCK
__device__ unsigned long long gram_clock[3];
extern "C" __attribute__((visibility("default"))) int ate_gram_clock_read(void* host) {
  return (int)hipMemcpyFromSymbol(host, HIP_SYMBOL(gram_clock), sizeof(gram_clock));
}
extern "C" __attribute__((visibility("default"))) int ate_gram_clock_reset() {
  static unsigned long long z[3];
  return (int)hipMemcpyToSymbol(HIP_SYMBOL(gram_clock), z, sizeof(z));
}
#endif

template <bool BYTES, int SCHED>
__global__ __launch_bounds__(512) void gram_bf16_pair_kernel(
    const bf16_t* __restrict__ X, int64_t cs, int64_t bs, const int4* __restrict__ tiles, int ntiles,
    const Chunk* __restrict__ chunks, int nchunks, float* __restrict__ slab,
    const uint8_t* __restrict__ X8, int prio) {
  __shared__ __attribute__((aligned(16))) bf16_t lds[PAIR_LDS];
#ifdef GRAM_CLOCK
  const unsigned long long gc0 = clock64(), gw0 = wall_clock64();
#endif
  const int L = xcd_remap(blockIdx.x, gridDim.x);
  const int c = L / ntiles, t = L % ntiles;
  ATE_DASSERT(c < nchunks && t < ntiles);
  const Chunk ch = chunks[c];
  const int4 tl = tiles[t];
  const int type = tl.z;
  ATE_DASSERT(ch.row0 >= 0 && ch.row0 <= ch.row1 && ch.row0 % GK == 0 && ch.row1 % GK == 0);
  ATE_DASSERT(tl.x >= 0 && tl.y >= tl.x && type >= 0 && type <= 2);
  const bool haveB = type != 2;
  const int a0 = tl.x * GT, b0 = tl.y * GT;
  const int wid = threadIdx.x >> 6;
  const bool tri = type != 0 && wid >= 4;
  const int region = type == 0 ? 0 : (tri ? (wid - 4) >> 1 : wid >> 1);
  const int half = type == 0 ? 0 : (wid & 1);
  const bool idle = type == 2 && region == 1;
  int arow0, bcol0;
  if (type == 0) { arow0 = (wid >> 2) * 128; bcol0 = (wid & 3) * 64; }
  else if (!tri) { arow0 = 0; bcol0 = 128 + half * 64; }
  else { arow0 = half * 128; bcol0 = half * 128; }
  const int abuf = type == 0 ? 0 : region;
  const int bbuf = type == 0 ? 1 : region;
  constexpr int RS = PairRole<PAIR_RECT_D0>::NB, TS = PairRole<PAIR_TRI>::NB;
  const int base = type == 0 ? wid * 32 : tri ? 4 * RS + (wid - 4) * TS : wid * RS;
  float* out = slab + ((int64_t)c * ntiles + t) * (PAIR_SLOTS * 256) + (int64_t)base * 256;
  if ((prio == 1 || (prio == 2 && type != 0)) &&
      __builtin_amdgcn_readfirstlane(threadIdx.x) >= 256)
    __builtin_amdgcn_s_setprio(1);
  const bool by = BYTES && (type == 0 ? (wid & 3) >= 2 : region == 1 && (!tri || half == 1));
  ATE_DASSERT(!BYTES || (X8 != nullptr && ntiles == 2 && b0 == 256));
  constexpr bool STAG = (SCHED & SCHED_STAGGER) != 0;
#define PAIR_WAVE(M, B, L) pair_wave<M, BYTES, B, L, SCHED != SCHED_LOCKSTEP>(                      \
      X, cs, bs, a0, b0, haveB, idle, abuf, bbuf, arow0, bcol0, ch, lds, out, X8)
#define PAIR_WAVE_BY(M, L) do { if (by) PAIR_WAVE(M, BYTES, L); else PAIR_WAVE(M, false, L); } while (0)
  if (tri) PAIR_WAVE_BY(PAIR_TRI, STAG);
  else if (type == 0) {
    if (STAG && __builtin_amdgcn_readfirstlane(wid) >= 4) PAIR_WAVE_BY(PAIR_RECT, STAG);
    else PAIR_WAVE_BY(PAIR_RECT, false);
  }
  else if (half == 0) PAIR_WAVE_BY(PAIR_RECT_D0, false);
  else PAIR_WAVE_BY(PAIR_RECT_D1, false);
#undef PAIR_WAVE_BY
#undef PAIR_WAVE
#ifdef GRAM_CLOCK
  __syncthreads();
  if (threadIdx.x == 0) {
    atomicAdd(&gram_clock[0], (unsigned long long)(clock64() - gc0));
    atomicAdd(&gram_clock[1], (unsigned long long)(wall_clock64() - gw0));
    atomicAdd(&gram_clock[2], 1ull);
  }
#endif
}

__device__ __forceinline__ void gram_limbs(double v, long long& hi, long long& lo) {
  const double x = v * 16777216.0;
  const double h = floor(x);
  hi = (long long)h;
  lo = (long long)rint((x - h) * 4294967296.0);
}

__global__ void gram_pair_reduce_kernel(const float* __restrict__ slab, const int2* __restrict__ blocks,
                                        int ntiles, int slots, const int* __restrict__ seg_chunk0,
                                        int nseg, int P, double* __restrict__ G,
                                        long long* __restrict__ Gx, int byte0) {
  const int64_t per = (int64_t)ntiles * slots * 256;
  const int64_t total = (int64_t)nseg * per;
  for (int64_t e = blockIdx.x * (int64_t)blockDim.x + threadIdx.x; e < total;
       e += (int64_t)gridDim.x * blockDim.x) {
    const int s = (int)(e / per);
    const int64_t rem = e % per;
    const int tb = (int)(rem >> 8);
    const int ln = (int)(rem & 255) >> 2;
    const int r = ((ln >> 4) << 2) | (int)(rem & 3), cl = ln & 15;
    const int2 bl = blocks[tb];
    if (bl.x < 0) continue;
    if (bl.x == bl.y && r > cl) continue;
    const int c0 = seg_chunk0[s], c1 = seg_chunk0[s + 1];
    const float* src = slab + rem;
    const int a = bl.x * 16 + r, b = bl.y * 16 + cl;
    ATE_DASSERT(s < nseg && c0 >= 0 && c0 <= c1 && a >= 0 && a < P && b >= 0 && b < P);
    const double sc = (a >= byte0 ? 2.0 : 1.0) * (b >= byte0 ? 2.0 : 1.0);
    if (Gx) {
      long long hs = 0, ls = 0;
      int ci = c0;
      for (; ci + 8 <= c1; ci += 8) {
        float v[8];
#pragma unroll
        for (int u = 0; u < 8; ++u) v[u] = src[(int64_t)(ci + u) * per];
#pragma unroll
        for (int u = 0; u < 8; ++u) {
          long long h, l;
          gram_limbs((double)v[u] * sc, h, l);
          hs += h;
          ls += l;
        }
      }
      for (; ci < c1; ++ci) {
        long long h, l;
        gram_limbs((double)src[(int64_t)ci * per] * sc, h, l);
        hs += h;
        ls += l;
      }
      const int64_t PP = (int64_t)nseg * P * P;
      long long* Xs = Gx + (int64_t)s * P * P;
      Xs[(int64_t)a * P + b] = hs;
      Xs[(int64_t)b * P + a] = hs;
      Xs[PP + (int64_t)a * P + b] = ls;
      Xs[PP + (int64_t)b * P + a] = ls;
      continue;
    }
    double acc = 0.0;
    int ci = c0;
    for (; ci + 8 <= c1; ci += 8) {
      float v[8];
#pragma unroll
      for (int u = 0; u < 8; ++u) v[u] = src[(int64_t)(ci + u) * per];
#pragma unroll
      for (int u = 0; u < 8; ++u) acc += (double)v[u];
    }
    for (; ci < c1; ++ci) acc += (double)src[(int64_t)ci * per];
    acc *= sc;
    double* Gs = G + (int64_t)s * P * P;
    Gs[(int64_t)a * P + b] = acc;
    Gs[(int64_t)b * P + a] = acc;
  }
}

#define PAIR_SCHEDS(F) F(0) F(1)
#define PAIR_SHAPE(S)                                                                     \
  static ate::KernelShapeReg ate_kshape_pair_##S(                                         \
      (const void*)(gram_bf16_pair_kernel<false, S>), "gram_bf16_pair_kernel<sched " #S ">", 512, 0); \
  static ate::KernelShapeReg ate_kshape_pair8_##S(                                        \
      (const void*)(gram_bf16_pair_kernel<true, S>), "gram_bf16_pair_kernel<bytes, sched " #S ">", 512, 0);
PAIR_SCHEDS(PAIR_SHAPE)
#undef PAIR_SHAPE
ATE_KERNEL_SHAPE("gram_bf16_256_kernel", 512, 0, gram_bf16_256_kernel)
ATE_KERNEL_SHAPE("gram_bf16_kernel", 256, 0, gram_bf16_kernel)

ATE_API int ate_gram_bf16_pair(const void* X, int64_t cs, int64_t bs, int P, const void* tiles, int ntiles,
                               const void* blocks, const void* chunks, int nchunks,
                               const void* seg_chunk0, int nseg, void* slab, void* G, int what,
                               void* Gx, const void* X8, int sched, int prio, void* stream) {
  if (P % (2 * GT) || what < 1 || what > 3) return -1;
  if (X8 != nullptr && (P != 512 || ntiles != 2)) return -1;
  if (sched != SCHED_LOCKSTEP && cs >= ((int64_t)1 << 28)) return -1;
  if (prio < 0) prio = sched == SCHED_STAGGER ? 0 : GRAM_PRIO;
  if (prio > 2) return -1;
  hipStream_t s = (hipStream_t)stream;
  if (what & 1) {
    switch (sched) {
#define PAIR_LAUNCH(S)                                                                        \
  case S:                                                                                     \
    if (X8 != nullptr)                                                                        \
      ATE_LAUNCH((gram_bf16_pair_kernel<true, S>), dim3(nchunks * ntiles), dim3(512), 0, s,   \
                 (const bf16_t*)X, cs, bs, (const int4*)tiles, ntiles, (const Chunk*)chunks,  \
                 nchunks, (float*)slab, (const uint8_t*)X8, prio);                            \
    else                                                                                      \
      ATE_LAUNCH((gram_bf16_pair_kernel<false, S>), dim3(nchunks * ntiles), dim3(512), 0, s,  \
                 (const bf16_t*)X, cs, bs, (const int4*)tiles, ntiles, (const Chunk*)chunks,  \
                 nchunks, (float*)slab, (const uint8_t*)nullptr, prio);                       \
    break;
      PAIR_SCHEDS(PAIR_LAUNCH)
#undef PAIR_LAUNCH
      default: return -1;
    }
    ATE_CHECK_LAUNCH();
  }
  if (what & 2) {
    const int64_t total = (int64_t)nseg * ntiles * PAIR_SLOTS * 256;
    ATE_LAUNCH(gram_pair_reduce_kernel, dim3(grid_for(total, 256, 4096)), dim3(256), 0, s,
                       (const float*)slab, (const int2*)blocks, ntiles, PAIR_SLOTS,
                       (const int*)seg_chunk0, nseg, P, (double*)G, (long long*)Gx,
                       X8 != nullptr ? PAIR_BYTE0 : P);
    ATE_CHECK_LAUNCH();
  }
  return 0;
}

constexpr int FT = 64;
constexpr int FK = 16;

typedef __attribute__((ext_vector_type(4))) double f64x4;
template <typename T> struct AccT;
template <> struct AccT<float> { typedef f32x4 type; };
template <> struct AccT<double> { typedef f64x4 type; };

__device__ __forceinline__ f32x4 mfma_16x16x4(float a, float b, f32x4 c) {
  return __builtin_amdgcn_mfma_f32_16x16x4f32(a, b, c, 0, 0, 0);
}
__device__ __forceinline__ f64x4 mfma_16x16x4(double a, double b, f64x4 c) {
  return __builtin_amdgcn_mfma_f64_16x16x4f64(a, b, c, 0, 0, 0);
}
__device__ __forceinline__ int acc_row(float, int lane, int r) { return (lane >> 4) * 4 + r; }
__device__ __forceinline__ int acc_row(double, int lane, int r) { return (lane >> 4) + 4 * r; }

template <typename T>
__global__ __launch_bounds__(256) void gram_small_kernel(
    const T* __restrict__ X, int64_t ld, const T* __restrict__ w,
    const int2* __restrict__ tiles, int ntiles, const Chunk* __restrict__ chunks, int nchunks,
    T* __restrict__ slab, const int* __restrict__ done) {
  if (done && *done) return;
  typedef typename AccT<T>::type acc_t;
  __shared__ T lds[2][FT * (FK + 1)];
  const int L = xcd_remap(blockIdx.x, gridDim.x);
  const int c = L / ntiles, t = L % ntiles;
  const Chunk ch = chunks[c];
  const int2 tl = tiles[t];
  const int a0 = tl.x * FT, b0 = tl.y * FT;
  const int tid = threadIdx.x, lane = tid & 63, wid = tid >> 6;
  const int wr = wid >> 1, wc = wid & 1;
  acc_t acc[2][2];
#pragma unroll
  for (int i = 0; i < 2; ++i)
#pragma unroll
    for (int j = 0; j < 2; ++j) acc[i][j] = acc_t{0, 0, 0, 0};

  for (int64_t i0 = ch.row0; i0 < ch.row1; i0 += FK) {
#pragma unroll
    for (int r = 0; r < 4; ++r) {
      int idx = r * 256 + tid, col = idx >> 4, row = idx & 15;
      int64_t gi = i0 + row;
      T wv = w ? w[gi] : T(1);
      lds[0][col * (FK + 1) + row] = X[(int64_t)(a0 + col) * ld + gi] * wv;
      lds[1][col * (FK + 1) + row] = X[(int64_t)(b0 + col) * ld + gi];
    }
    __syncthreads();
#pragma unroll
    for (int k4 = 0; k4 < FK; k4 += 4) {
      T af[2], bfv[2];
#pragma unroll
      for (int m = 0; m < 2; ++m)
        af[m] = lds[0][(wr * 32 + m * 16 + (lane & 15)) * (FK + 1) + k4 + (lane >> 4)];
#pragma unroll
      for (int n = 0; n < 2; ++n)
        bfv[n] = lds[1][(wc * 32 + n * 16 + (lane & 15)) * (FK + 1) + k4 + (lane >> 4)];
#pragma unroll
      for (int m = 0; m < 2; ++m)
#pragma unroll
        for (int n = 0; n < 2; ++n) acc[m][n] = mfma_16x16x4(af[m], bfv[n], acc[m][n]);
    }
    __syncthreads();
  }
  T* out = slab + ((int64_t)c * ntiles + t) * (FT * FT);
#pragma unroll
  for (int m = 0; m < 2; ++m)
#pragma unroll
    for (int n = 0; n < 2; ++n)
#pragma unroll
      for (int r = 0; r < 4; ++r) {
        int row = wr * 32 + m * 16 + acc_row(T(0), lane, r);
        int col = wc * 32 + n * 16 + (lane & 15);
        out[row * FT + col] = acc[m][n][r];
      }
}

template <typename S>
__global__ void gram_reduce_kernel(const S* __restrict__ slab, int T, const int2* __restrict__ tiles,
                                   int ntiles, const int* __restrict__ seg_chunk0, int nseg, int P,
                                   double* __restrict__ G, const int* __restrict__ done,
                                   long long* __restrict__ Gx) {
  if (done && *done) return;
  const int tt = T * T;
  const int64_t total = (int64_t)nseg * ntiles * tt;
  for (int64_t e = blockIdx.x * (int64_t)blockDim.x + threadIdx.x; e < total;
       e += (int64_t)gridDim.x * blockDim.x) {
    int s = (int)(e / ((int64_t)ntiles * tt));
    int rem = (int)(e % ((int64_t)ntiles * tt));
    int t = rem / tt, ij = rem % tt;
    if (tiles[t].x == tiles[t].y && ij / T > ij % T) continue;
    if (Gx) {
      long long hs = 0, ls = 0;
      for (int c = seg_chunk0[s]; c < seg_chunk0[s + 1]; ++c) {
        long long h, l;
        gram_limbs((double)slab[((int64_t)c * ntiles + t) * tt + ij], h, l);
        hs += h;
        ls += l;
      }
      const int a = tiles[t].x * T + ij / T, b = tiles[t].y * T + ij % T;
      const int64_t PP = (int64_t)nseg * P * P;
      long long* Xs = Gx + (int64_t)s * P * P;
      Xs[(int64_t)a * P + b] = hs;
      Xs[(int64_t)b * P + a] = hs;
      Xs[PP + (int64_t)a * P + b] = ls;
      Xs[PP + (int64_t)b * P + a] = ls;
      continue;
    }
    double acc = 0.0;
    for (int c = seg_chunk0[s]; c < seg_chunk0[s + 1]; ++c)
      acc += (double)slab[((int64_t)c * ntiles + t) * tt + ij];
    int a = tiles[t].x * T + ij / T, b = tiles[t].y * T + ij % T;
    double* Gs = G + (int64_t)s * P * P;
    Gs[(int64_t)a * P + b] = acc;
    Gs[(int64_t)b * P + a] = acc;
  }
}

ATE_API int ate_gram_bf16(const void* X, int64_t ld, int P, int tile,
                          const void* tiles, int ntiles, const void* chunks, int nchunks,
                          const void* seg_chunk0, int nseg, void* slab, void* G, void* Gx,
                          void* stream) {
  hipStream_t s = (hipStream_t)stream;
  int nwg = nchunks * ntiles;
  if (tile == GT) {
    if (P % GT) return -1;
    ATE_LAUNCH(gram_bf16_256_kernel, dim3(nwg), dim3(512), 0, s, (const bf16_t*)X, ld,
                       (const int2*)tiles, ntiles, (const Chunk*)chunks, nchunks, (float*)slab);
  } else if (tile == BT) {
    if (P % BT) return -1;
    ATE_LAUNCH(gram_bf16_kernel, dim3(nwg), dim3(256), 0, s, (const bf16_t*)X, ld,
                       (const int2*)tiles, ntiles, (const Chunk*)chunks, nchunks, (float*)slab);
  } else {
    return -1;
  }
  ATE_CHECK_LAUNCH();
  int64_t total = (int64_t)nseg * ntiles * tile * tile;
  ATE_LAUNCH(gram_reduce_kernel<float>, dim3(grid_for(total, 256, 4096)), dim3(256), 0, s,
                     (const float*)slab, tile, (const int2*)tiles, ntiles, (const int*)seg_chunk0,
                     nseg, P, (double*)G, (const int*)nullptr, (long long*)Gx);
  ATE_CHECK_LAUNCH();
  return 0;
}

template <typename T>
static int gram_small(const void* X, int64_t ld, int P, const void* w, const void* tiles,
                      int ntiles, const void* chunks, int nchunks, const void* seg_chunk0,
                      int nseg, void* slab, void* G, const void* done, void* Gx, void* stream) {
  if (P % FT) return -1;
  hipStream_t s = (hipStream_t)stream;
  int nwg = nchunks * ntiles;
  ATE_LAUNCH(gram_small_kernel<T>, dim3(nwg), dim3(256), 0, s, (const T*)X, ld,
                     (const T*)w, (const int2*)tiles, ntiles, (const Chunk*)chunks, nchunks,
                     (T*)slab, (const int*)done);
  ATE_CHECK_LAUNCH();
  int64_t total = (int64_t)nseg * ntiles * FT * FT;
  ATE_LAUNCH(gram_reduce_kernel<T>, dim3(grid_for(total, 256, 4096)), dim3(256), 0, s,
                     (const T*)slab, FT, (const int2*)tiles, ntiles, (const int*)seg_chunk0,
                     nseg, P, (double*)G, (const int*)done, (long long*)Gx);
  ATE_CHECK_LAUNCH();
  return 0;
}

ATE_API int ate_gram_f32(const void* X, int64_t ld, int P, const void* w, const void* tiles,
                         int ntiles, const void* chunks, int nchunks, const void* seg_chunk0,
                         int nseg, void* slab, void* G, const void* done, void* Gx, void* stream) {
  return gram_small<float>(X, ld, P, w, tiles, ntiles, chunks, nchunks, seg_chunk0, nseg, slab, G,
                        done, Gx, stream);
}

ATE_API int ate_gram_f64(const void* X, int64_t ld, int P, const void* w, const void* tiles,
                         int ntiles, const void* chunks, int nchunks, const void* seg_chunk0,
                         int nseg, void* slab, void* G, const void* done, void* Gx, void* stream) {
  return gram_small<double>(X, ld, P, w, tiles, ntiles, chunks, nchunks, seg_chunk0, nseg, slab, G,
                        done, Gx, stream);
}

ATE_API int ate_gram_tile_sizes(int* bf16_tile, int* bf16_kstep, int* f32_tile, int* f32_kstep) {
  *bf16_tile = BT; *bf16_kstep = BK; *f32_tile = FT; *f32_kstep = FK;
  return 0;
}
```

Measured before the change: 2.333 billion rows/s.

## Pack binary Gram columns into 1-bit blocks and expand in-register for MFMA

Adds a bit-packed copy of the binary columns (1 bit per value instead of 1 byte), built once after data generation by a new pack kernel. A new Gram pair kernel variant stages only 1 KB of bits per 64-row block into LDS and expands bits to bf16 (value 2.0) in registers with perm/shift/mask, compensating with a 0.5 scale in the reduce. The aim is to cut HBM and LDS traffic for the binary tail of the panel. In exchange it adds ALU expansion work, new hand-tuned schedule barriers, and an extra buffer that must be kept in sync through graph capture.

```diff
diff --git a/ate_replication_causalml_amd/_native.py b/ate_replication_causalml_amd/_native.py
--- a/ate_replication_causalml_amd/_native.py
+++ b/ate_replication_causalml_amd/_native.py
@@ -52,6 +52,7 @@
 _SIGS = {
     "ate_gram_bf16": "pliipipipipppp",
     "ate_gram_bf16_pair": "pllipippipippippiip",
+    "ate_gram_bf16_pair_bits": "pllipippipippippiip",
     "ate_last_error": "pi",
     "ate_last_stale_error": "pi",
     "ate_clear_errors": "",
@@ -115,6 +116,7 @@
     "ate_lognet_path_groups": "iplpiipipipppdpdiippppppppp",
     "ate_lognet_cvloss_set": "iplpiipipipppipp",
     "ate_dgp_fill": "iplllllp" + "uiipppp",
+    "ate_dgp_pack_bits": "plpp",
     "ate_sel_block_rows": "",
     "ate_sel_gen_count": "upilllpp",
     "ate_sel_gen_flags": "upillpp",
diff --git a/ate_replication_causalml_amd/data/device_dgp.py b/ate_replication_causalml_amd/data/device_dgp.py
--- a/ate_replication_causalml_amd/data/device_dgp.py
+++ b/ate_replication_causalml_amd/data/device_dgp.py
@@ -31,6 +31,48 @@
 
 BYTE_COL0 = 384
 BYTE_PANEL = os.environ.get("ATE_PANEL_BYTES", "1") == "1"
+BIT_PANEL = os.environ.get("ATE_PANEL_BITS", "1") == "1"
+BITS_BLOCK = 1024
+
+
+def bits1_index(col, row):
+    col, row = np.broadcast_arrays(np.asarray(col), np.asarray(row))
+    lane = ((row >> 3) & 3) * 16 + (col & 15)
+    byte = (col >> 6) * 512 + lane * 8 + ((col >> 4) & 3) * 2 + (row & 1)
+    bit = (row >> 5) * 4 + ((row >> 1) & 3)
+    return byte, bit
+
+
+def pack_bits_block(block) -> np.ndarray:
+    b = np.asarray(block) != 0
+    if b.shape != (128, 64):
+        raise ValueError("a bit block is 128 columns x 64 rows")
+    byte, bit = bits1_index(np.arange(128)[:, None], np.arange(64)[None, :])
+    out = np.zeros(BITS_BLOCK, dtype=np.uint8)
+    np.bitwise_or.at(out, byte[b], (1 << bit[b]).astype(np.uint8))
+    return out
+
+
+def unpack_bits_block(image) -> np.ndarray:
+    im = np.asarray(image, dtype=np.uint8).reshape(BITS_BLOCK)
+    byte, bit = bits1_index(np.arange(128)[:, None], np.arange(64)[None, :])
+    return (im[byte] >> bit.astype(np.uint8)) & 1
+
+
+def pack_bits(bytes8: torch.Tensor) -> torch.Tensor:
+    if not bytes8.is_cuda or not bytes8.is_contiguous() or tuple(bytes8.shape[1:]) != (128, 64):
+        raise ValueError("pack_bits needs a contiguous [nblk, 128, 64] uint8 tensor on the GPU")
+    out = torch.empty((bytes8.shape[0], BITS_BLOCK), dtype=torch.uint8, device=bytes8.device)
+    _native.call("ate_dgp_pack_bits", bytes8.data_ptr(), bytes8.shape[0], out.data_ptr(),
+                 torch.cuda.current_stream().cuda_stream)
+    return out
+
+
+def unpack_bits(bits1: torch.Tensor) -> torch.Tensor:
+    byte, bit = bits1_index(np.arange(128)[:, None], np.arange(64)[None, :])
+    byte = torch.from_numpy(byte.reshape(-1).astype(np.int64)).to(bits1.device)
+    bit = torch.from_numpy(bit.reshape(-1).astype(np.uint8)).to(bits1.device)
+    return ((bits1[:, byte] >> bit) & 1).reshape(-1, 128, 64)
 
 
 def _binary_names(p: int) -> set:
@@ -141,6 +183,8 @@
                          *pan.strides(), int(r0), cnt, g0, gp, seed, p_extra, int(hi_lo),
                          pblk.ctypes.data, None if pcol is None else pcol.data_ptr(),
                          None if pcol is None else pan.bytes8.data_ptr(), s)
+        if pcol is not None and BIT_PANEL:
+            pan.bits1 = pack_bits(pan.bytes8)
     else:
         cm = torch.zeros((pan.P, pan.ld), dtype=pan.data.dtype) if blocked else pan.data
         for k, ((g0, cnt), (r0, _)) in enumerate(zip(slices, pan.seg_bounds)):
diff --git a/ate_replication_causalml_amd/ops/gram.py b/ate_replication_causalml_amd/ops/gram.py
--- a/ate_replication_causalml_amd/ops/gram.py
+++ b/ate_replication_causalml_amd/ops/gram.py
@@ -250,11 +250,14 @@
     s = _stream()
     if X.dtype == torch.bfloat16 and pl.pair:
         cs, bs = panel.strides()
-        x8 = getattr(panel, "bytes8", None)
-        _native.call("ate_gram_bf16_pair", X.data_ptr(), cs, bs, panel.P, pl.tiles.data_ptr(),
+        x8 = getattr(panel, "bytes8", None) if BYTE_COLS else None
+        x1 = getattr(panel, "bits1", None) if x8 is not None else None
+        _native.call("ate_gram_bf16_pair" if x1 is None else "ate_gram_bf16_pair_bits",
+                     X.data_ptr(), cs, bs, panel.P, pl.tiles.data_ptr(),
                      pl.ntiles, pl.blocks.data_ptr(), pl.chunks.data_ptr(), pl.nchunks,
                      pl.seg_chunk0.data_ptr(), panel.nseg, pl.slab.data_ptr(), G.data_ptr(),
-                     _STAGES[stage], Gx, None if x8 is None or not BYTE_COLS else x8.data_ptr(),
+                     _STAGES[stage], Gx,
+                     x1.data_ptr() if x1 is not None else None if x8 is None else x8.data_ptr(),
                      _sched_for(cs), GRAM_PRIO, s)
         return pl.Gx if exact else G
     if stage == "reduce":
diff --git a/ate_replication_causalml_amd/ops/panel.py b/ate_replication_causalml_amd/ops/panel.py
--- a/ate_replication_causalml_amd/ops/panel.py
+++ b/ate_replication_causalml_amd/ops/panel.py
@@ -29,6 +29,7 @@
     blocked: bool = False
     exact_block: int = 0
     bytes8: torch.Tensor | None = None
+    bits1: torch.Tensor | None = None
 
     @property
     def P(self):
diff --git a/ate_replication_causalml_amd/utils/graphs.py b/ate_replication_causalml_amd/utils/graphs.py
--- a/ate_replication_causalml_amd/utils/graphs.py
+++ b/ate_replication_causalml_amd/utils/graphs.py
@@ -199,7 +199,8 @@
         if not isinstance(x, torch.Tensor):
             k += (x.n, tuple(sorted(x.cols.items())), tuple(map(tuple, x.seg_bounds)),
                   tuple(int(c) for c in x.seg_nreal), bool(getattr(x, "identity", False)),
-                  getattr(x, "bytes8", None) is not None)
+                  getattr(x, "bytes8", None) is not None,
+                  getattr(x, "bits1", None) is not None)
         key.append(k)
     return tuple(key)
 
@@ -216,6 +217,8 @@
                 _data(s).copy_(_data(x))
                 if getattr(x, "bytes8", None) is not None:
                     s.bytes8.copy_(x.bytes8)
+                if getattr(x, "bits1", None) is not None:
+                    s.bits1.copy_(x.bits1)
 
     def __call__(self, inputs):
         self.load(inputs)
@@ -295,6 +298,8 @@
                         _data(s).copy_(_data(x))
                         if getattr(x, "bytes8", None) is not None:
                             s.bytes8.copy_(x.bytes8)
+                        if getattr(x, "bits1", None) is not None:
+                            s.bits1.copy_(x.bits1)
                 g = _Captured(body, static, static_args, warmup=1)
             except Exception as e:
                 print(f"[graphs] {name}: capture failed, running eagerly: {e}", flush=True)
diff --git a/csrc/dgp.hip b/csrc/dgp.hip
--- a/csrc/dgp.hip
+++ b/csrc/dgp.hip
@@ -107,6 +107,32 @@
 __device__ __forceinline__ int x8_pos(int64_t i) {
   const int r = (int)(i & 63);
   return ((r >> 3) & 3) * 16 + (r >> 5) * 8 + (r & 7);
+}
+
+__device__ __forceinline__ int x1_byte(int cb, int row) {
+  const int l = ((row >> 3) & 3) * 16 + (cb & 15);
+  return (cb >> 6) * 512 + l * 8 + ((cb >> 4) & 3) * 2 + (row & 1);
+}
+__device__ __forceinline__ int x1_bit(int row) { return (row >> 5) * 4 + ((row >> 1) & 3); }
+
+__global__ void dgp_pack_bits_kernel(const uint8_t* __restrict__ X8, int64_t nblk,
+                                     uint8_t* __restrict__ X1) {
+  const int64_t total = nblk * 512;
+  for (int64_t e = blockIdx.x * (int64_t)blockDim.x + threadIdx.x; e < total;
+       e += (int64_t)gridDim.x * blockDim.x) {
+    const int64_t blk = e >> 9;
+    const int cb = (int)(e & 511) >> 2, r = (int)(e & 3);
+    const uint4 v = *reinterpret_cast<const uint4*>(X8 + blk * (128 * 64) + cb * 64 + r * 16);
+    const uint32_t w[4] = {v.x, v.y, v.z, v.w};
+    uint32_t h = 0;
+#pragma unroll
+    for (int k = 0; k < 16; ++k) {
+      const int row = (k >> 3) * 32 + r * 8 + (k & 7);
+      const uint32_t b = (w[k >> 2] >> ((k & 3) * 8)) & 0xFFu;
+      h |= (b != 0 ? 1u : 0u) << ((row & 1) * 8 + x1_bit(row));
+    }
+    *reinterpret_cast<uint16_t*>(X1 + blk * 1024 + x1_byte(cb, r * 8)) = (uint16_t)h;
+  }
 }
 
 template <typename T>
@@ -288,6 +314,14 @@
   return 0;
 }
 
+ATE_API int ate_dgp_pack_bits(const void* X8, int64_t nblk, void* X1, void* stream) {
+  if (nblk <= 0) return 0;
+  ATE_LAUNCH(dgp_pack_bits_kernel, dim3(grid_for(nblk * 512, 256, 8192)), dim3(256), 0,
+                     (hipStream_t)stream, (const uint8_t*)X8, nblk, (uint8_t*)X1);
+  ATE_CHECK_LAUNCH();
+  return 0;
+}
+
 ATE_API int ate_sel_block_rows() { return SEL_BR; }
 
 ATE_API int ate_sel_gen_count(uint64_t seed, const void* params, int last, int64_t b0, int64_t nblk,
diff --git a/csrc/gram.hip b/csrc/gram.hip
--- a/csrc/gram.hip
+++ b/csrc/gram.hip
@@ -200,9 +200,16 @@
   static constexpr int NB = TRI ? 36 : 32;
 };
 
-template <int MODE>
+template <int MODE, bool COLS = false>
 __device__ __forceinline__ void pair_mfma(f32x4* acc, const bf16x8* af, const bf16x8* bfr) {
-  if constexpr (MODE != PAIR_TRI) {
+  if constexpr (MODE == PAIR_TRI && COLS) {
+#pragma unroll
+    for (int n = 0; n < 8; ++n)
+#pragma unroll
+      for (int m = 0; m <= n; ++m)
+        acc[tri_index(m, n)] = __builtin_amdgcn_mfma_f32_16x16x32_bf16(
+            af[m], af[n], acc[tri_index(m, n)], 0, 0, 0);
+  } else if constexpr (MODE != PAIR_TRI) {
 #pragma unroll
     for (int m = 0; m < 8; ++m)
 #pragma unroll
@@ -229,14 +236,35 @@
 }
 constexpr int PAIR_BYTE0 = 384;
 
+template <int HW>
+__device__ __forceinline__ uint32_t bits_rep(uint32_t d) {
+  return __builtin_amdgcn_perm(0u, d, HW ? 0x02030302u : 0x00010100u);
+}
+template <int H>
+__device__ __forceinline__ bf16x8 bits_to_bf16x8(uint32_t w) {
+  uint4 v;
+  v.x = (w << (14 - 4 * H)) & 0x40004000u;
+  v.y = (w << (13 - 4 * H)) & 0x40004000u;
+  v.z = (w << (12 - 4 * H)) & 0x40004000u;
+  v.w = (w << (11 - 4 * H)) & 0x40004000u;
+  return __builtin_bit_cast(bf16x8, v);
+}
+constexpr int COL_BF16 = 0, COL_BYTES = 1, COL_BITS = 2;
+template <int MASK, int N>
+__device__ __forceinline__ void sched_group() {
+  if constexpr (N > 0) __builtin_amdgcn_sched_group_barrier(MASK, N, 0);
+}
+
 constexpr int SCHED_LOCKSTEP = 0, SCHED_STAGGER = 1;
 
-template <int MODE, bool BYTES, bool BY, bool LATE, bool SADDR>
+template <int MODE, int CM, bool BY, bool LATE, bool SADDR>
 __device__ __forceinline__ void pair_wave(const bf16_t* __restrict__ X, int64_t cs, int64_t bs, int a0,
                                           int b0, bool haveB, bool idle, int abuf, int bbuf,
                                           int arow0, int bcol0, const Chunk& ch,
                                           bf16_t* lds_raw, float* __restrict__ out,
                                           const uint8_t* __restrict__ X8) {
+  constexpr bool BYTES = CM != COL_BF16;
+  constexpr bool BITS = CM == COL_BITS;
   constexpr bool TRI = PairRole<MODE>::TRI;
   constexpr int NB = PairRole<MODE>::NB;
   const int tid = threadIdx.x, lane = tid & 63, wid = tid >> 6;
@@ -246,7 +274,8 @@
   bf16_t (*lds)[2][GT * GK] = reinterpret_cast<bf16_t (*)[2][GT * GK]>(lds_raw);
   const int wu = __builtin_amdgcn_readfirstlane(wid);
   const uint32_t voff_ = (uint32_t)(((lane >> 3) * cs + (((lane & 7) ^ (lane >> 3)) << 3)) * 2);
-  const uint32_t voff8_ = (uint32_t)((lane >> 2) * GK + (((lane & 3) ^ ((lane >> 3) & 2)) << 4));
+  const uint32_t voff8_ = BITS ? (uint32_t)(lane * 16)
+                               : (uint32_t)((lane >> 2) * GK + (((lane & 3) ^ ((lane >> 3) & 2)) << 4));
   auto stage = [&](int st, int64_t i0) {
     if constexpr (SADDR) {
       gptr_t Xk0 = (gptr_t) reinterpret_cast<const char*>(X + (i0 >> 6) * bs);
@@ -268,10 +297,35 @@
           const int q = wu * 2 + r;
           glds16(Xk0 + (int64_t)(b0 + q * 8) * cs * 2 + voff, &lds[st][1][q * 8 * GK]);
         }
-        glds16((gptr_t) reinterpret_cast<const char*>(X8) + (i0 >> 6) * (128 * GK) + wu * 1024 + voff8,
-               reinterpret_cast<bf16_t*>(reinterpret_cast<uint8_t*>(&lds[st][1][128 * GK]) +
-                                         wu * 1024));
-      }
+        if constexpr (BITS) {
+          if (wu == 0)
+            glds16((gptr_t) reinterpret_cast<const char*>(X8) + (i0 >> 6) * 1024 + voff8,
+                   &lds[st][1][128 * GK]);
+        } else {
+          glds16((gptr_t) reinterpret_cast<const char*>(X8) + (i0 >> 6) * (128 * GK) + wu * 1024 + voff8,
+                 reinterpret_cast<bf16_t*>(reinterpret_cast<uint8_t*>(&lds[st][1][128 * GK]) +
+                                           wu * 1024));
+        }
+      }
+      return;
+    }
+    if constexpr (BITS) {
+      const bf16_t* Xk0 = X + (i0 >> 6) * bs;
+#pragma unroll
+      for (int r = 0; r < 4; ++r) {
+        const int q = wid * 4 + r;
+        const int col = q * 8 + (lane >> 3);
+        const int cc = (lane & 7) ^ (col & 7);
+        glds16(Xk0 + cc * 8 + (int64_t)(a0 + col) * cs, &lds[st][0][q * 8 * GK]);
+      }
+#pragma unroll
+      for (int r = 0; r < 2; ++r) {
+        const int q = wid * 2 + r;
+        const int col = q * 8 + (lane >> 3);
+        const int cc = (lane & 7) ^ (col & 7);
+        glds16(Xk0 + cc * 8 + (int64_t)(b0 + col) * cs, &lds[st][1][q * 8 * GK]);
+      }
+      if (wu == 0) glds16(X8 + (i0 >> 6) * 1024 + lane * 16, &lds[st][1][128 * GK]);
       return;
     }
     if constexpr (BYTES) {
@@ -316,6 +370,14 @@
     const int slot = (lane >> 4) ^ ((cb >> 1) & 2);
     return *reinterpret_cast<const uint4*>(b8 + cb * GK + slot * 16);
   };
+  auto bits4 = [&](const bf16_t* P_, int col0, uint32_t* w) {
+    const uint8_t* b1 = reinterpret_cast<const uint8_t*>(P_ + 128 * GK);
+    const uint2 q = *reinterpret_cast<const uint2*>(b1 + ((col0 - 128) >> 6) * 512 + lane * 8);
+    w[0] = bits_rep<0>(q.x);
+    w[1] = bits_rep<1>(q.x);
+    w[2] = bits_rep<0>(q.y);
+    w[3] = bits_rep<1>(q.y);
+  };
   const int64_t nsteps = (ch.row1 - ch.row0) / GK;
   if (nsteps > 0) stage(0, ch.row0);
   __builtin_amdgcn_s_waitcnt(0x0F70);
@@ -335,16 +397,51 @@
     const bf16_t* Bs = lds[cur][bbuf];
     if constexpr (LATE) {
       bf16x8 na[8], nb[TRI ? 1 : 4];
-      uint4 raw[BY ? (TRI ? 8 : 4) : 1];
+      uint4 raw[BY && !BITS ? (TRI ? 8 : 4) : 1];
+      uint32_t bw[BY && BITS ? (TRI ? 8 : 4) : 1];
       const int c0 = lane >> 4, c1 = 4 + (lane >> 4);
       if (!idle) {
-        if constexpr (BY && !TRI) {
-#pragma unroll
-          for (int n = 0; n < 4; ++n) raw[n] = raw16(Bs, bcol0 + n * 16 + (lane & 15));
+        if constexpr (BY && BITS && !TRI) {
+          bits4(Bs, bcol0, bw);
 #pragma unroll
           for (int m = 0; m < 8; ++m) na[m] = frag(As, arow0 + m * 16 + (lane & 15), c0);
           pair_mfma<MODE>(acc, ha, hb);
 #pragma unroll
+          for (int i = 0; i < 9; ++i) {
+            __builtin_amdgcn_sched_group_barrier(0x008, 1, 0);
+            __builtin_amdgcn_sched_group_barrier(0x100, 1, 0);
+          }
+          __builtin_amdgcn_sched_group_barrier(0x008, 1, 0);
+          __builtin_amdgcn_sched_group_barrier(0x002, 4, 0);
+          __builtin_amdgcn_sched_group_barrier(0x008, NB - 10, 0);
+        } else if constexpr (BY && BITS) {
+          bits4(As, arow0, bw);
+          bits4(As, arow0 + 64, bw + 4);
+#pragma unroll
+          for (int m = 0; m < 8; ++m) na[m] = bits_to_bf16x8<0>(bw[m]);
+          pair_mfma<MODE>(acc, ha, ha);
+#pragma unroll
+          for (int i = 0; i < 2; ++i) {
+            __builtin_amdgcn_sched_group_barrier(0x008, 1, 0);
+            __builtin_amdgcn_sched_group_barrier(0x100, 1, 0);
+          }
+#pragma unroll
+          for (int i = 0; i < 32; ++i) {
+            __builtin_amdgcn_sched_group_barrier(0x008, 1, 0);
+            __builtin_amdgcn_sched_group_barrier(0x002, 2, 0);
+          }
+#pragma unroll
+          for (int i = 0; i < 2; ++i) {
+            __builtin_amdgcn_sched_group_barrier(0x008, 1, 0);
+            __builtin_amdgcn_sched_group_barrier(0x002, 4, 0);
+          }
+        } else if constexpr (BY && !TRI) {
+#pragma unroll
+          for (int n = 0; n < 4; ++n) raw[n] = raw16(Bs, bcol0 + n * 16 + (lane & 15));
+#pragma unroll
+          for (int m = 0; m < 8; ++m) na[m] = frag(As, arow0 + m * 16 + (lane & 15), c0);
+          pair_mfma<MODE>(acc, ha, hb);
+#pragma unroll
           for (int i = 0; i < 12; ++i) {
             __builtin_amdgcn_sched_group_barrier(0x008, 1, 0);
             __builtin_amdgcn_sched_group_barrier(0x100, 1, 0);
@@ -393,7 +490,42 @@
       }
       if (s + 1 < nsteps) stage(cur ^ 1, ch.row0 + (s + 1) * GK);
       if (!idle) {
-        if constexpr (BY && !TRI) {
+        if constexpr (BY && BITS && !TRI) {
+#pragma unroll
+          for (int m = 0; m < 8; ++m) ha[m] = frag(As, arow0 + m * 16 + (lane & 15), c1);
+#pragma unroll
+          for (int n = 0; n < 4; ++n) nb[n] = bits_to_bf16x8<0>(bw[n]);
+#pragma unroll
+          for (int n = 0; n < 4; ++n) hb[n] = bits_to_bf16x8<1>(bw[n]);
+          pair_mfma<MODE>(acc, na, nb);
+          __builtin_amdgcn_sched_group_barrier(0x002, 8, 0);
+#pragma unroll
+          for (int i = 0; i < 3; ++i) {
+            __builtin_amdgcn_sched_group_barrier(0x008, 1, 0);
+            __builtin_amdgcn_sched_group_barrier(0x002, 8, 0);
+          }
+#pragma unroll
+          for (int i = 0; i < 8; ++i) {
+            __builtin_amdgcn_sched_group_barrier(0x008, 1, 0);
+            __builtin_amdgcn_sched_group_barrier(0x100, 1, 0);
+          }
+#pragma unroll
+          for (int i = 0; i < 16; ++i) {
+            __builtin_amdgcn_sched_group_barrier(0x008, 1, 0);
+            __builtin_amdgcn_sched_group_barrier(0x002, 2, 0);
+          }
+          __builtin_amdgcn_sched_group_barrier(0x008, NB - 27, 0);
+        } else if constexpr (BY && BITS) {
+#pragma unroll
+          for (int m = 0; m < 8; ++m) ha[m] = bits_to_bf16x8<1>(bw[m]);
+          pair_mfma<MODE>(acc, na, na);
+#pragma unroll
+          for (int i = 0; i < 32; ++i) {
+            __builtin_amdgcn_sched_group_barrier(0x008, 1, 0);
+            __builtin_amdgcn_sched_group_barrier(0x002, 2, 0);
+          }
+          __builtin_amdgcn_sched_group_barrier(0x008, NB - 32, 0);
+        } else if constexpr (BY && !TRI) {
 #pragma unroll
           for (int m = 0; m < 8; ++m) ha[m] = frag(As, arow0 + m * 16 + (lane & 15), c1);
 #pragma unroll
@@ -455,7 +587,55 @@
     } else {
       if (s + 1 < nsteps) stage(cur ^ 1, ch.row0 + (s + 1) * GK);
       if (!idle) {
-        if constexpr (BY && !TRI) {
+        if constexpr (BY && BITS && !TRI) {
+          bf16x8 af[2][8];
+          uint32_t w4[4];
+          bits4(Bs, bcol0, w4);
+#pragma unroll
+          for (int kk = 0; kk < 2; ++kk) {
+            const int cc = kk * 4 + (lane >> 4);
+#pragma unroll
+            for (int m = 0; m < 8; ++m) af[kk][m] = frag(As, arow0 + m * 16 + (lane & 15), cc);
+          }
+          bf16x8 b0v[4], b1v[4];
+#pragma unroll
+          for (int n = 0; n < 4; ++n) b0v[n] = bits_to_bf16x8<0>(w4[n]);
+#pragma unroll
+          for (int n = 0; n < 4; ++n) b1v[n] = bits_to_bf16x8<1>(w4[n]);
+          pair_mfma<MODE>(acc, af[0], b0v);
+          pair_mfma<MODE>(acc, af[1], b1v);
+          __builtin_amdgcn_sched_group_barrier(0x100, 9, 0);
+          __builtin_amdgcn_sched_group_barrier(0x002, 36, 0);
+#pragma unroll
+          for (int i = 0; i < 8; ++i) {
+            __builtin_amdgcn_sched_group_barrier(0x008, 1, 0);
+            __builtin_amdgcn_sched_group_barrier(0x100, 1, 0);
+          }
+#pragma unroll
+          for (int i = 0; i < 16; ++i) {
+            __builtin_amdgcn_sched_group_barrier(0x008, 1, 0);
+            __builtin_amdgcn_sched_group_barrier(0x002, 2, 0);
+          }
+          __builtin_amdgcn_sched_group_barrier(0x008, 2 * NB - 24, 0);
+        } else if constexpr (BY && BITS) {
+          uint32_t w8[8];
+          bits4(As, arow0, w8);
+          bits4(As, arow0 + 64, w8 + 4);
+          bf16x8 f0[8], f1[8];
+#pragma unroll
+          for (int m = 0; m < 8; ++m) f0[m] = bits_to_bf16x8<0>(w8[m]);
+#pragma unroll
+          for (int m = 0; m < 8; ++m) f1[m] = bits_to_bf16x8<1>(w8[m]);
+          pair_mfma<MODE, true>(acc, f0, f0);
+          pair_mfma<MODE, true>(acc, f1, f1);
+          __builtin_amdgcn_sched_group_barrier(0x100, 2, 0);
+          __builtin_amdgcn_sched_group_barrier(0x002, 16, 0);
+#define TRI_COL(C) sched_group<0x008, 1>(); sched_group<0x002, 8>(); sched_group<0x008, C>();
+          TRI_COL(0) TRI_COL(1) TRI_COL(2) TRI_COL(3) TRI_COL(4) TRI_COL(5) TRI_COL(6) TRI_COL(7)
+          TRI_COL(0) TRI_COL(1) TRI_COL(2) TRI_COL(3) TRI_COL(4) TRI_COL(5) TRI_COL(6)
+#undef TRI_COL
+          __builtin_amdgcn_sched_group_barrier(0x008, 8, 0);
+        } else if constexpr (BY && !TRI) {
           bf16x8 af[2][8];
           uint4 braw[4];
 #pragma unroll
@@ -567,7 +747,7 @@
 }
 #endif
 
-template <bool BYTES, int SCHED>
+template <int CM, int SCHED>
 __global__ __launch_bounds__(512) void gram_bf16_pair_kernel(
     const bf16_t* __restrict__ X, int64_t cs, int64_t bs, const int4* __restrict__ tiles, int ntiles,
     const Chunk* __restrict__ chunks, int nchunks, float* __restrict__ slab,
@@ -603,10 +783,11 @@
   if ((prio == 1 || (prio == 2 && type != 0)) &&
       __builtin_amdgcn_readfirstlane(threadIdx.x) >= 256)
     __builtin_amdgcn_s_setprio(1);
+  constexpr bool BYTES = CM != COL_BF16;
   const bool by = BYTES && (type == 0 ? (wid & 3) >= 2 : region == 1 && (!tri || half == 1));
   ATE_DASSERT(!BYTES || (X8 != nullptr && ntiles == 2 && b0 == 256));
   constexpr bool STAG = (SCHED & SCHED_STAGGER) != 0;
-#define PAIR_WAVE(M, B, L) pair_wave<M, BYTES, B, L, SCHED != SCHED_LOCKSTEP>(                      \
+#define PAIR_WAVE(M, B, L) pair_wave<M, CM, B, L, SCHED != SCHED_LOCKSTEP>(                         \
       X, cs, bs, a0, b0, haveB, idle, abuf, bbuf, arow0, bcol0, ch, lds, out, X8)
 #define PAIR_WAVE_BY(M, L) do { if (by) PAIR_WAVE(M, BYTES, L); else PAIR_WAVE(M, false, L); } while (0)
   if (tri) PAIR_WAVE_BY(PAIR_TRI, STAG);
@@ -638,7 +819,7 @@
 __global__ void gram_pair_reduce_kernel(const float* __restrict__ slab, const int2* __restrict__ blocks,
                                         int ntiles, int slots, const int* __restrict__ seg_chunk0,
                                         int nseg, int P, double* __restrict__ G,
-                                        long long* __restrict__ Gx, int byte0) {
+                                        long long* __restrict__ Gx, int byte0, double bsc) {
   const int64_t per = (int64_t)ntiles * slots * 256;
   const int64_t total = (int64_t)nseg * per;
   for (int64_t e = blockIdx.x * (int64_t)blockDim.x + threadIdx.x; e < total;
@@ -655,7 +836,7 @@
     const float* src = slab + rem;
     const int a = bl.x * 16 + r, b = bl.y * 16 + cl;
     ATE_DASSERT(s < nseg && c0 >= 0 && c0 <= c1 && a >= 0 && a < P && b >= 0 && b < P);
-    const double sc = (a >= byte0 ? 2.0 : 1.0) * (b >= byte0 ? 2.0 : 1.0);
+    const double sc = (a >= byte0 ? bsc : 1.0) * (b >= byte0 ? bsc : 1.0);
     if (Gx) {
       long long hs = 0, ls = 0;
       int ci = c0;
@@ -705,39 +886,42 @@
 #define PAIR_SCHEDS(F) F(0) F(1)
 #define PAIR_SHAPE(S)                                                                     \
   static ate::KernelShapeReg ate_kshape_pair_##S(                                         \
-      (const void*)(gram_bf16_pair_kernel<false, S>), "gram_bf16_pair_kernel<sched " #S ">", 512, 0); \
+      (const void*)(gram_bf16_pair_kernel<COL_BF16, S>), "gram_bf16_pair_kernel<sched " #S ">", 512, 0); \
   static ate::KernelShapeReg ate_kshape_pair8_##S(                                        \
-      (const void*)(gram_bf16_pair_kernel<true, S>), "gram_bf16_pair_kernel<bytes, sched " #S ">", 512, 0);
+      (const void*)(gram_bf16_pair_kernel<COL_BYTES, S>), "gram_bf16_pair_kernel<bytes, sched " #S ">", 512, 0); \
+  static ate::KernelShapeReg ate_kshape_pair1_##S(                                        \
+      (const void*)(gram_bf16_pair_kernel<COL_BITS, S>), "gram_bf16_pair_kernel<bits, sched " #S ">", 512, 0);
 PAIR_SCHEDS(PAIR_SHAPE)
 #undef PAIR_SHAPE
 ATE_KERNEL_SHAPE("gram_bf16_256_kernel", 512, 0, gram_bf16_256_kernel)
 ATE_KERNEL_SHAPE("gram_bf16_kernel", 256, 0, gram_bf16_kernel)
 
-ATE_API int ate_gram_bf16_pair(const void* X, int64_t cs, int64_t bs, int P, const void* tiles, int ntiles,
-                               const void* blocks, const void* chunks, int nchunks,
-                               const void* seg_chunk0, int nseg, void* slab, void* G, int what,
-                               void* Gx, const void* X8, int sched, int prio, void* stream) {
+static int gram_pair(int cm, const void* X, int64_t cs, int64_t bs, int P, const void* tiles,
+                     int ntiles, const void* blocks, const void* chunks, int nchunks,
+                     const void* seg_chunk0, int nseg, void* slab, void* G, int what, void* Gx,
+                     const void* X8, int sched, int prio, void* stream) {
   if (P % (2 * GT) || what < 1 || what > 3) return -1;
+  if ((cm != COL_BF16) != (X8 != nullptr)) return -1;
   if (X8 != nullptr && (P != 512 || ntiles != 2)) return -1;
   if (sched != SCHED_LOCKSTEP && cs >= ((int64_t)1 << 28)) return -1;
   if (prio < 0) prio = sched == SCHED_STAGGER ? 0 : GRAM_PRIO;
   if (prio > 2) return -1;
   hipStream_t s = (hipStream_t)stream;
   if (what & 1) {
+#define PAIR_LAUNCH_CM(C, S)                                                                  \
+  ATE_LAUNCH((gram_bf16_pair_kernel<C, S>), dim3(nchunks * ntiles), dim3(512), 0, s,          \
+             (const bf16_t*)X, cs, bs, (const int4*)tiles, ntiles, (const Chunk*)chunks,      \
+             nchunks, (float*)slab, (const uint8_t*)X8, prio)
     switch (sched) {
 #define PAIR_LAUNCH(S)                                                                        \
   case S:                                                                                     \
-    if (X8 != nullptr)                                                                        \
-      ATE_LAUNCH((gram_bf16_pair_kernel<true, S>), dim3(nchunks * ntiles), dim3(512), 0, s,   \
-                 (const bf16_t*)X, cs, bs, (const int4*)tiles, ntiles, (const Chunk*)chunks,  \
-                 nchunks, (float*)slab, (const uint8_t*)X8, prio);                            \
-    else                                                                                      \
-      ATE_LAUNCH((gram_bf16_pair_kernel<false, S>), dim3(nchunks * ntiles), dim3(512), 0, s,  \
-                 (const bf16_t*)X, cs, bs, (const int4*)tiles, ntiles, (const Chunk*)chunks,  \
-                 nchunks, (float*)slab, (const uint8_t*)nullptr, prio);                       \
+    if (cm == COL_BITS) PAIR_LAUNCH_CM(COL_BITS, S);                                          \
+    else if (cm == COL_BYTES) PAIR_LAUNCH_CM(COL_BYTES, S);                                   \
+    else PAIR_LAUNCH_CM(COL_BF16, S);                                                         \
     break;
       PAIR_SCHEDS(PAIR_LAUNCH)
 #undef PAIR_LAUNCH
+#undef PAIR_LAUNCH_CM
       default: return -1;
     }
     ATE_CHECK_LAUNCH();
@@ -747,10 +931,27 @@
     ATE_LAUNCH(gram_pair_reduce_kernel, dim3(grid_for(total, 256, 4096)), dim3(256), 0, s,
                        (const float*)slab, (const int2*)blocks, ntiles, PAIR_SLOTS,
                        (const int*)seg_chunk0, nseg, P, (double*)G, (long long*)Gx,
-                       X8 != nullptr ? PAIR_BYTE0 : P);
+                       X8 != nullptr ? PAIR_BYTE0 : P, cm == COL_BITS ? 0.5 : 2.0);
     ATE_CHECK_LAUNCH();
   }
   return 0;
+}
+
+ATE_API int ate_gram_bf16_pair(const void* X, int64_t cs, int64_t bs, int P, const void* tiles, int ntiles,
+                               const void* blocks, const void* chunks, int nchunks,
+                               const void* seg_chunk0, int nseg, void* slab, void* G, int what,
+                               void* Gx, const void* X8, int sched, int prio, void* stream) {
+  return gram_pair(X8 != nullptr ? COL_BYTES : COL_BF16, X, cs, bs, P, tiles, ntiles, blocks,
+                   chunks, nchunks, seg_chunk0, nseg, slab, G, what, Gx, X8, sched, prio, stream);
+}
+
+ATE_API int ate_gram_bf16_pair_bits(const void* X, int64_t cs, int64_t bs, int P, const void* tiles,
+                                    int ntiles, const void* blocks, const void* chunks, int nchunks,
+                                    const void* seg_chunk0, int nseg, void* slab, void* G, int what,
+                                    void* Gx, const void* X1, int sched, int prio, void* stream) {
+  if (X1 == nullptr) return -1;
+  return gram_pair(COL_BITS, X, cs, bs, P, tiles, ntiles, blocks, chunks, nchunks, seg_chunk0,
+                   nseg, slab, G, what, Gx, X1, sched, prio, stream);
 }
 
 constexpr int FT = 64;
```

Result: faster. 2.411 billion rows/s, median of 6 (+3.3%).
